# shubhamchandak94/HARC

Hardware: AMD Instinct MI355X
Metric: Mreads/s reorder+encode, 100 bp (higher is better)
Workload: dtype u64 (2-bit packed bases, XOR+popcount)

## Files before the change

harc_amd/csrc/stage1.hip:

```cpp
#include "devutil.h"
#include <stdlib.h>
#include <type_traits>

struct S1Args {
    int L, maxmatch, thresh, maxsearch, Lp;
    int ds[2], de[2], kbits[2];
    uint32_t N, K;
    const uint64_t *reads;
    HashSlot *slots[2];
    uint64_t cap[2];
    const uint32_t *ids[2];
    int firstmax;
    const uint32_t *bloom[2]; uint32_t bloom_lines; int bloom_nwin[2]; uint32_t bloom_mmask;
    const uint2 *largetab;
    uint64_t *mirror;
    unsigned long long *claimed;
    uint32_t *bid;
    ChainHdr *hdr;
    uint4 *cnt;
    uint2 *steps;
    uint8_t *need;
    uint32_t *seedbuf;
    uint32_t *needrank;
    uint32_t *rmeta;
// ... 318 lines not shown
    const bool have = i < nbins;
    auto slot_of = [&](uint32_t k) -> uint64_t { return q[k] - (uint64_t)n + (uint64_t)k; };
    const uint32_t b0 = blockIdx.x * blockDim.x, b1 = b0 + blockDim.x < nbins ? b0 + blockDim.x : nbins;
    bool tiled = false; uint64_t lo = 0, hi = 0;
    if (pass == 0 && fill && b0 < nbins) {
        lo = b0 ? slot_of(b0 - 1) + 1 : 0;
        const uint64_t last = slot_of(b1 - 1);
        if (lo < cap) {
            hi = (last >= cap || b1 == nbins || slot_of(b1) >= cap) ? cap : last + 1;
            tiled = hi - lo <= TP_SPAN;
        }
    }
    if (tiled) {
        const uint4 z = make_uint4(0u, 0u, 0u, 0u);
        for (uint32_t j = threadIdx.x; j < (uint32_t)(hi - lo); j += blockDim.x) tile[j] = z;
        __syncthreads();
    }
    uint64_t sl = have ? slot_of(i) : 0;
    bool mine = have;
    if (mine && pass == 0 && sl >= cap && blockIdx.x + 64 < gridDim.x) { atomicAdd(nbins_p + 1, 1u); mine = false; }
    if (mine && (pass == 1) != (sl >= cap)) mine = false;
    if (mine) {
        const uint32_t st = binstart[i];
        const uint64_t key = skeys[st];
        uint32_t ovf = 0;
        if (pass == 0 && (sl & 3) == 0 && (uint64_t)i + 4 < (uint64_t)nbins) {
            const uint64_t s3 = slot_of(i + 3);
            if (s3 == sl + 3 && (bucket_slot(skeys[binstart[i + 4]], cap) >> 2) <= (sl >> 2)) ovf = SLOT_OVF;
        }
        if (pass == 0 && fill && !tiled) {
            const uint4 z = make_uint4(0u, 0u, 0u, 0u);
            for (uint64_t x = i ? slot_of(i - 1) + 1 : 0; x < sl; x++) *reinterpret_cast<uint4 *>(&slots[x]) = z;
            if (i + 1 == nbins || slot_of(i + 1) >= cap)
                for (uint64_t x = sl + 1; x < cap; x++) *reinterpret_cast<uint4 *>(&slots[x]) = z;
        }
        const uint32_t en = (i + 1 < nbins) ? binstart[i + 1] : n;
        const uint32_t cnt = en - st;
        if (cnt > SLOT_CNT_MASK) atomicAdd(nbins_p + 1, 1u);
        else {
            const unsigned long long meta = cnt == 1 ? ((unsigned long long)sids[st] | ((unsigned long long)(1u | SLOT_EMB) << 32))
                                                     : ((unsigned long long)st | ((unsigned long long)((cnt & SLOT_CNT_MASK) | ((bigthresh && cnt > bigthresh) ? SLOT_BIG : 0u)) << 32));
            if (pass == 1) {
                for (uint64_t bb = bucket_slot(key, cap) >> 2; bb < (cap >> 2); bb++) atomicOr(&slots[4 * bb].count, SLOT_OVF);
                sl = 0;
                for (;;) {
                    unsigned long long *mp = reinterpret_cast<unsigned long long *>(&slots[sl]) + 1;
                    if (atomicCAS(mp, 0ULL, meta) == 0ULL) break;
                    if ((sl & 3) == 3) atomicOr(&slots[sl - 3].count, SLOT_OVF);
                    if (++sl == cap) sl = 0;
                }
                slots[sl].key = key;
            } else {
                uint4 w; w.x = (uint32_t)key; w.y = (uint32_t)(key >> 32); w.z = (uint32_t)meta; w.w = (uint32_t)(meta >> 32) | ovf;
                if (tiled) tile[sl - lo] = w; else *reinterpret_cast<uint4 *>(&slots[sl]) = w;
            }
            if (large_list && cnt > HARC_LARGEBIN) {
                const unsigned int at = atomicAdd(large_n, 1u);
                if (at < large_max) large_list[at] = ((unsigned long long)sl << 1) | large_tag;
            }
        }
    }
    if (tiled) {
        __syncthreads();
        for (uint32_t j = threadIdx.x; j < (uint32_t)(hi - lo); j += blockDim.x) *reinterpret_cast<uint4 *>(&slots[lo + j]) = tile[j];
    }
}

__global__ __launch_bounds__(256) void k_s1_bloom_tile(const uint64_t *pk, uint32_t n, uint64_t nwords, uint32_t *bloom)
{
    __shared__ uint32_t tile[BL_TILE_WORDS];
    __shared__ uint32_t bounds[2];
    const uint32_t part = blockIdx.x;
    for (uint32_t j = threadIdx.x; j < BL_TILE_WORDS; j += 256) tile[j] = 0u;
    if (threadIdx.x < 2) {
        const uint64_t want = (uint64_t)part + threadIdx.x, pmask = ((uint64_t)1 << BL_PART_BITS) - 1;
        uint32_t lo = 0, hi = n;
        while (lo < hi) { const uint32_t mid = lo + (hi - lo) / 2; if ((pk[mid] & pmask) < want) lo = mid + 1; else hi = mid; }
        bounds[threadIdx.x] = lo;
    }
    __syncthreads();
    for (uint32_t i = bounds[0] + threadIdx.x; i < bounds[1]; i += 256) {
        const uint32_t v = (uint32_t)(pk[i] >> BL_PART_BITS);
        atomicOr(&tile[v >> 10], (1u << ((v >> 5) & 31u)) | (1u << (v & 31u)));
    }
    __syncthreads();
    const uint64_t base = (uint64_t)part * BL_TILE_WORDS;
    for (uint32_t j = threadIdx.x; j < BL_TILE_WORDS; j += 256) if (base + j < nwords) bloom[base + j] = tile[j];
}
int harc_bitmap_from_items(harc_amd_ctx *c, const uint64_t *items, uint64_t *tmp, size_t n, uint64_t nwords, uint32_t *bitmap)
{
    const uint64_t ntiles64 = (nwords + BL_TILE_WORDS - 1) / BL_TILE_WORDS;
    if (ntiles64 + 1 >= (1ull << BL_PART_BITS) || n > 0xFFFFFFFFull) { harc_set_error("bitmap of %llu words / %zu items: too large for the tiled build", (unsigned long long)nwords, n); return HARC_AMD_EINVAL; }
    const uint32_t ntiles = (uint32_t)ntiles64;
    if (ntiles == 0) return HARC_AMD_OK;
    unsigned tb = 1; while (((uint64_t)1 << tb) <= ntiles) tb++;
    RC_TRY(prim_sort_keys_u64(c, items, tmp, n, tb));
    hipLaunchKernelGGL(k_s1_bloom_tile, dim3(ntiles), dim3(256), 0, c->stream, (const uint64_t *)tmp, (uint32_t)n, nwords, bitmap);
    HIP_TRY(hipGetLastError());
    return HARC_AMD_OK;
}
__global__ void k_s1_bloom_diff(const uint32_t *a, const uint32_t *b, uint64_t nwords, unsigned long long *ndiff)
{
    const uint64_t i = harc_gid();
    const bool d = i < nwords && a[i] != b[i];
    const unsigned long long m = __ballot(d);
    if ((threadIdx.x & 63) == 0 && m) atomicAdd(ndiff, (unsigned long long)__popcll(m));
}
__global__ void k_s1_bloom_set(const uint64_t *keys, uint32_t n, uint32_t *bloom, uint32_t nlines, int nwin, uint32_t mmask)
{
    const uint32_t i = harc_gid32();
    if (i >= n) return;
    uint32_t w, m;
    bloom_pos(keys[i], key_scramble(keys[i]), nlines, nwin, mmask, &w, &m);
    if ((bloom[w] & m) != m) atomicOr(&bloom[w], m);
}

__global__ void k_init_chains(S1Args s)
{
    const uint32_t c = harc_gid32();
    if (c >= s.K) return;
    ChainHdr h; memset(&h, 0, sizeof h);
    const uint32_t step = s.N / s.K;
    const bool act = s.N > 0 && (c == 0 || step > 0);
    if (act) {
        const uint32_t seed = c * step;
        atomicOr(&s.claimed[seed >> 6], 1ULL << (seed & 63));
        h.cur = seed; h.prev = seed; h.flags = CH_ACTIVE | CH_PREVUNM; h.mode = 2;
    }
    s.hdr[c] = h;
    s.cst2[c] = make_uint2(act ? 1u : 0u, 0u);
    s.need[c] = 0;
    s.pg_cur[c] = c * PG_CHUNK;
    for (uint32_t k = 0; k < PG_CHUNK; k++) s.pg_hdr[(size_t)c * PG_CHUNK + k] = make_uint2(c, k);
    if (c == 0) *s.pg_count = s.K * PG_CHUNK;
}

template <int W, bool INLDS> struct ConsState {
    static constexpr int CT = (W + 1) / 2;
    static constexpr int LP = 64 * CT;
    uint4 qr[INLDS ? 1 : CT];
    uint4 *ql;
    int v[CT];
    int base;
    __device__ __forceinline__ uint4 getq(int t) const { if constexpr (INLDS) return ql[64 * t]; else return qr[t]; }
    __device__ __forceinline__ void setq(int t, const uint4 &q) { if constexpr (INLDS) ql[64 * t] = q; else qr[t] = q; }
};
__device__ __forceinline__ int argmax4(const uint4 &q)
{
    uint32_t mx = 0; int ind = 0;
    if (q.x > mx) { mx = q.x; ind = 0; }
    if (q.y > mx) { mx = q.y; ind = 1; }
    if (q.z > mx) { mx = q.z; ind = 2; }
    if (q.w > mx) { mx = q.w; ind = 3; }
    return ind;
}
template <int W> __device__ __forceinline__ int oriented_base(const uint64_t (&rw)[W], int L, int rev, int i)
{
    const int sc = rev ? (L - 1 - i) : i;
    const int pc = (int)((sel0<W>(rw, sc >> 5) >> (2 * (sc & 31))) & 3);
    const int b = ((pc & 1) << 1) | (pc >> 1);
    return rev ? 3 - b : b;
}
template <int W, bool I> __device__ __forceinline__ void cons_reset(ConsState<W, I> &st, const uint64_t (&rw)[W], int L, int lane)
{
    st.base = 0;
#pragma unroll
    for (int t = 0; t < ConsState<W, I>::CT; t++) {
        const int i = lane + 64 * t;
        int b = 0; uint4 q = make_uint4(0, 0, 0, 0);
        if (i < L) { b = oriented_base<W>(rw, L, 0, i); q.x = (b == 0); q.y = (b == 1); q.z = (b == 2); q.w = (b == 3); }
        st.setq(t, q); st.v[t] = b;
    }
}
template <int W, bool I> __device__ __forceinline__ void cons_update(ConsState<W, I> &st, const uint64_t (&rw)[W], int L, int rev, int shift, int lane)
{
    constexpr int LP = ConsState<W, I>::LP;
    int nb = st.base + shift; if (nb >= LP) nb -= LP;
#pragma unroll
    for (int t = 0; t < ConsState<W, I>::CT; t++) {
        const int p = lane + 64 * t;
        int oldl = p - st.base; if (oldl < 0) oldl += LP;
        int newl = p - nb; if (newl < 0) newl += LP;
        uint4 q = st.getq(t); int v = 0;
        if (newl < L) {
            const int b = oriented_base<W>(rw, L, rev, newl);
            if (oldl < L && oldl >= shift) { q.x += (b == 0); q.y += (b == 1); q.z += (b == 2); q.w += (b == 3); v = argmax4(q); }
            else { q.x = (b == 0); q.y = (b == 1); q.z = (b == 2); q.w = (b == 3); v = b; }
        } else q = make_uint4(0, 0, 0, 0);
        st.setq(t, q); st.v[t] = v;
    }
    st.base = nb;
}
template <int W, bool I> __device__ __forceinline__ void cons_load(ConsState<W, I> &st, const uint4 *src, int L, int lane, uint32_t fmt)
{
    st.base = 0;
#pragma unroll
    for (int t = 0; t < ConsState<W, I>::CT; t++) {
        const int i = lane + 64 * t;
        uint4 q = make_uint4(0, 0, 0, 0); int v = 0;
        if (i < L) {
            if (fmt == 2u) q = src[i];
            else if (fmt == 1u) { const uint2 p = reinterpret_cast<const uint2 *>(src)[i]; q = make_uint4(p.x & 0xFFFFu, p.x >> 16, p.y & 0xFFFFu, p.y >> 16); }
            else { const uint32_t p = reinterpret_cast<const uint32_t *>(src)[i]; q = make_uint4(p & 0xFFu, (p >> 8) & 0xFFu, (p >> 16) & 0xFFu, p >> 24); }
            v = argmax4(q);
        }
        st.setq(t, q); st.v[t] = v;
    }
}
template <int W, bool I> __device__ __forceinline__ uint32_t cons_store(const ConsState<W, I> &st, uint4 *dst, int L, int lane)
{
    constexpr int LP = ConsState<W, I>::LP;
    uint32_t mx = 0;
#pragma unroll
    for (int t = 0; t < ConsState<W, I>::CT; t++) {
        int l = lane + 64 * t - st.base; if (l < 0) l += LP;
        if (l < L) { const uint4 q = st.getq(t); const uint32_t a = q.x > q.y ? q.x : q.y, b = q.z > q.w ? q.z : q.w; const uint32_t m = a > b ? a : b; mx = m > mx ? m : mx; }
    }
    const uint32_t fmt = __ballot(mx > 0xFFFFu) != 0 ? 2u : (__ballot(mx > 0xFFu) != 0 ? 1u : 0u);
#pragma unroll
    for (int t = 0; t < ConsState<W, I>::CT; t++) {
        int l = lane + 64 * t - st.base; if (l < 0) l += LP;
        if (l < L) {
            const uint4 q = st.getq(t);
            if (fmt == 2u) dst[l] = q;
            else if (fmt == 1u) reinterpret_cast<uint2 *>(dst)[l] = make_uint2(q.x | (q.y << 16), q.z | (q.w << 16));
            else reinterpret_cast<uint32_t *>(dst)[l] = q.x | (q.y << 8) | (q.z << 16) | (q.w << 24);
        }
    }
    return fmt;
}
template <int W, bool I> __device__ __forceinline__ void cons_pack(const ConsState<W, I> &st, int L, int lane, uint64_t (&ref)[W])
{
    constexpr int CT = ConsState<W, I>::CT, LP = ConsState<W, I>::LP, RW = 2 * CT;
    uint64_t ring[RW];
#pragma unroll
    for (int t = 0; t < CT; t++) {
        int l = lane + 64 * t - st.base; if (l < 0) l += LP;
        const bool valid = l < L;
        const int v = st.v[t];
        const unsigned long long b0 = __ballot(valid && (v >> 1)), b1 = __ballot(valid && (v & 1));
        ring[2 * t] = spread32(b0) | (spread32(b1) << 1);
        ring[2 * t + 1] = spread32(b0 >> 32) | (spread32(b1 >> 32) << 1);
    }
    const int sb = 2 * st.base, ws = sb >> 6, bs = sb & 63;
#pragma unroll
    for (int w = 0; w < W; w++) {
        int i0 = w + ws; if (i0 >= RW) i0 -= RW;
        int i1 = i0 + 1; if (i1 >= RW) i1 -= RW;
        const uint64_t lo = sel0<RW>(ring, i0), hi = sel0<RW>(ring, i1);
        ref[w] = (bs ? ((lo >> bs) | (hi << (64 - bs))) : lo) & lowmask_word(2 * L, w);
    }
}

#ifndef HARC_STEPS_WAVES
#define HARC_STEPS_WAVES 5
#endif
#ifndef HARC_COOP_WAVES
#define HARC_COOP_WAVES 4
#endif
#ifndef HARC_STEPS_WAVES_Q
#define HARC_STEPS_WAVES_Q 3
#endif
template <int W> struct StepsLds {
    static constexpr int NW = 2 * W;
    static constexpr int ROW = 3 * NW + 1;
    static constexpr int MROW = (NW + 3) & ~3;
};
#ifndef HARC_SEQ_SCAN
#define HARC_SEQ_SCAN 1
#endif
#ifndef HARC_SCAN_CH
#define HARC_SCAN_CH 1
#endif
#define HARC_WGCMD_BYTES 3584
#define HARC_SK_E 4
#ifndef HARC_SCAN_SKETCH
#define HARC_SCAN_SKETCH 1
#endif
#define HARC_OWN_SLOTS 128
#ifndef HARC_SEQ_OWNT
#define HARC_SEQ_OWNT 1
#endif
__device__ __forceinline__ void own_insert(uint32_t *tab, uint32_t id)
{
    uint32_t h = (id * 0x9E3779B1u) >> 25;
    while (tab[h] != HARC_NONE) h = (h + 1u) & (HARC_OWN_SLOTS - 1u);
    tab[h] = id;
}
__device__ __forceinline__ bool own_has(const uint32_t *tab, uint32_t id)
{
    uint32_t h = (id * 0x9E3779B1u) >> 25;
    for (;;) {
        const uint32_t v = tab[h];
        if (v == id) return true;
        if (v == HARC_NONE) return false;
        h = (h + 1u) & (HARC_OWN_SLOTS - 1u);
    }
}
static inline size_t steps_lds_bytes_coop(int W, int maxmatch, int nprobe)
{
    const int NW = 2 * W, ROW = 3 * NW + 1, MROW = (NW + 3) & ~3;
    return ((size_t)2 * maxmatch * MROW + (size_t)((2 * ROW + 3) & ~3) + (size_t)MROW + (size_t)8 * NW + (size_t)32 + (size_t)2 * nprobe + 8) * 4 + HARC_WGCMD_BYTES + 16;
}
static inline size_t steps_lds_bytes(int W, int maxmatch, int nprobe, bool seq = false)
{
    const int NW = 2 * W, ROW = 3 * NW + 1, MROW = (NW + 3) & ~3;
    return (size_t)4 * (64 * ((W + 1) / 2)) * 16 + ((size_t)2 * maxmatch * MROW + (size_t)4 * 2 * ROW + (size_t)4 * MROW + (size_t)4 * 8 * NW + (size_t)4 * 32 + (size_t)(seq ? 4 * HARC_OWN_SLOTS : 0) + (size_t)2 * nprobe + 8) * 4 + 32;
}
template <int W> __device__ __forceinline__ int ham_window(const uint32_t *row, int bitoff, const uint32_t *mrow, const uint32_t (&rd)[2 * W])
{
    constexpr int NW = 2 * W;
    const int i0 = bitoff >> 5, sh = bitoff & 31;
    uint32_t d[NW + 1];
#pragma unroll
    for (int k = 0; k <= NW; k++) d[k] = row[i0 + k];
    int hd = 0;
#pragma unroll
    for (int k = 0; k < NW; k++) hd += __popc((__builtin_amdgcn_alignbit(d[k + 1], d[k], sh) ^ rd[k]) & mrow[k]);
    return hd;
}
template <int W> __device__ __forceinline__ void load_read32(const uint64_t *reads, uint32_t rid, uint32_t (&rd)[2 * W])
{
    if (W % 2 == 0) {
        const uint4 *p = reinterpret_cast<const uint4 *>(reads + (size_t)rid * W);
#pragma unroll
        for (int q = 0; q < W / 2; q++) { const uint4 v = p[q]; rd[4 * q] = v.x; rd[4 * q + 1] = v.y; rd[4 * q + 2] = v.z; rd[4 * q + 3] = v.w; }
    } else {
        const uint2 *p = reinterpret_cast<const uint2 *>(reads + (size_t)rid * W);
#pragma unroll
        for (int q = 0; q < W; q++) { const uint2 v = p[q]; rd[2 * q] = v.x; rd[2 * q + 1] = v.y; }
    }
}
template <int W, bool I> __device__ __forceinline__ void cons_update_lds(ConsState<W, I> &st, const uint32_t *rdl, int L, int rev, int shift, int lane)
{
    constexpr int LP = ConsState<W, I>::LP;
    int nb = st.base + shift; if (nb >= LP) nb -= LP;
#pragma unroll
    for (int t = 0; t < ConsState<W, I>::CT; t++) {
        const int p = lane + 64 * t;
        int oldl = p - st.base; if (oldl < 0) oldl += LP;
        int newl = p - nb; if (newl < 0) newl += LP;
        uint4 q = st.getq(t); int v = 0;
        if (newl < L) {
            const int sc = rev ? (L - 1 - newl) : newl;
            const int pc = (int)((rdl[sc >> 4] >> (2 * (sc & 15))) & 3u);
            int b = ((pc & 1) << 1) | (pc >> 1);
            if (rev) b = 3 - b;
            if (oldl < L && oldl >= shift) { q.x += (b == 0); q.y += (b == 1); q.z += (b == 2); q.w += (b == 3); v = argmax4(q); }
            else { q.x = (b == 0); q.y = (b == 1); q.z = (b == 2); q.w = (b == 3); v = b; }
        } else q = make_uint4(0, 0, 0, 0);
        st.setq(t, q); st.v[t] = v;
    }
    st.base = nb;
}
template <int W, bool I> __device__ __forceinline__ void cons_reset_lds(ConsState<W, I> &st, const uint32_t *rdl, int L, int lane)
{
    st.base = 0;
#pragma unroll
    for (int t = 0; t < ConsState<W, I>::CT; t++) {
        const int i = lane + 64 * t;
        int b = 0; uint4 q = make_uint4(0, 0, 0, 0);
        if (i < L) {
            const int pc = (int)((rdl[i >> 4] >> (2 * (i & 15))) & 3u);
            b = ((pc & 1) << 1) | (pc >> 1);
            q.x = (b == 0); q.y = (b == 1); q.z = (b == 2); q.w = (b == 3);
        }
        st.setq(t, q); st.v[t] = b;
    }
}

template <int W, bool I> __device__ __forceinline__ void cons_rows(const ConsState<W, I> &st, int L, int lane, uint8_t *tmp, uint32_t *rowF, uint32_t *rowR)
{
    constexpr int CT = ConsState<W, I>::CT, LP = ConsState<W, I>::LP, NW = 2 * W;
#pragma unroll
    for (int t = 0; t < CT; t++) {
        int l = lane + 64 * t - st.base; if (l < 0) l += LP;
        if (l < L) {
            const int v = st.v[t];
            const int pc = ((v & 1) << 1) | (v >> 1);
            tmp[l] = (uint8_t)pc;
            tmp[16 * NW + (L - 1 - l)] = (uint8_t)(3 - pc);
        }
    }
    __builtin_amdgcn_fence(__ATOMIC_RELEASE, "wavefront");
    __builtin_amdgcn_wave_barrier();
    if (lane < 2 * NW) {
        const uint4 x = *reinterpret_cast<const uint4 *>(tmp + 16 * lane);
        auto pk = [](uint32_t b) -> uint32_t { b = (b | (b >> 6)) & 0x000F000Fu; return (b | (b >> 12)) & 0xFFu; };
        const uint32_t d = pk(x.x) | (pk(x.y) << 8) | (pk(x.z) << 16) | (pk(x.w) << 24);
        (lane < NW ? rowF + NW + lane : rowR + lane)[0] = d;
    }
    __builtin_amdgcn_fence(__ATOMIC_RELEASE, "wavefront");
    __builtin_amdgcn_wave_barrier();
}

template <int W> __device__ __forceinline__ void rows_from_read(const uint32_t *rdl, int L, int rev, int lane, uint32_t *rowF, uint32_t *rowR)
{
    constexpr int NW = 2 * W;
    int ln = lane; asm volatile("" : "+v"(ln));
    if (ln < 2 * NW) {
        const bool copy = ln < NW;
        const int k = copy ? ln : ln - NW;
        const int P = 2 * (L - 16 * k - 16), i0 = P >> 5;
        const int ia = i0 < 0 ? 0 : (i0 > NW - 1 ? NW - 1 : i0), ib = i0 + 1 < 0 ? 0 : (i0 + 1 > NW - 1 ? NW - 1 : i0 + 1);
        const uint32_t ra = rdl[copy ? k : ia], rb = rdl[ib];
        const uint32_t lo = (i0 >= 0 && i0 < NW) ? ra : 0u, hi = (i0 + 1 >= 0 && i0 + 1 < NW) ? rb : 0u;
        uint32_t w = __brev(__builtin_amdgcn_alignbit(hi, lo, P & 31));
        w = ((w & 0xAAAAAAAAu) >> 1) | ((w & 0x55555555u) << 1);
        const int vb = 2 * L - 32 * k;
        const uint32_t d = copy ? ra : (~w & (vb >= 32 ? 0xFFFFFFFFu : (vb <= 0 ? 0u : ((1u << vb) - 1u))));
        (copy != (rev != 0) ? rowF : rowR)[NW + k] = d;
    }
    __builtin_amdgcn_fence(__ATOMIC_RELEASE, "wavefront");
    __builtin_amdgcn_wave_barrier();
}
template <int W, bool I> __device__ __forceinline__ void cons_flush(ConsState<W, I> &st, const uint16_t *ps, int pend, int ptot, const uint32_t *rowF, int L, int lane)
{
    constexpr int LP = ConsState<W, I>::LP, CT = ConsState<W, I>::CT, NW = 2 * W;
    int nb = 0;
    if (ptot < L) { nb = st.base + ptot; if (nb >= LP) nb -= LP; }
    int ln = lane; asm volatile("" : "+v"(ln));
    int newl[CT], cnt[CT];
#pragma unroll
    for (int t = 0; t < CT; t++) { newl[t] = ln + 64 * t - nb; if (newl[t] < 0) newl[t] += LP; cnt[t] = 0; }
    for (int k = pend - 1; k >= 0; k--) {
        const int d = __builtin_amdgcn_readfirstlane(ptot - (int)ps[k]);
        if (d >= L) break;
#pragma unroll
        for (int t = 0; t < CT; t++) cnt[t] += (d < L - newl[t]) ? 1 : 0;
    }
#pragma unroll
    for (int t = 0; t < CT; t++) {
        uint4 q = make_uint4(0, 0, 0, 0); int v = 0;
        if (newl[t] < L) {
            const int pc = (int)((rowF[NW + (newl[t] >> 4)] >> (2 * (newl[t] & 15))) & 3u);
            v = ((pc & 1) << 1) | (pc >> 1);
            if (newl[t] + ptot < L) q = st.getq(t);
            const uint32_t c = (uint32_t)cnt[t];
            q.x += v == 0 ? c : 0u; q.y += v == 1 ? c : 0u; q.z += v == 2 ? c : 0u; q.w += v == 3 ? c : 0u;
        }
        st.setq(t, q); st.v[t] = v;
    }
    st.base = nb;
}

struct WgCmd {
    int op;
    int l, t, fast;
    uint32_t ids0, m0, cnt;
    uint32_t rot;
    unsigned long long grp;
    uint32_t found;
    uint32_t nc;
    unsigned long long hit[2][HARC_SCAN_CH][4];
    unsigned long long um[2][HARC_SCAN_CH][4];
    uint8_t mj[64], mdir[64];
    uint32_t own[64];
    unsigned long long um4[2][HARC_SK_E][4];
    uint32_t best[2][4];
    uint16_t queue[4][64 * HARC_SK_E];
};
struct WgResult { int besthit, fj, fdir; uint32_t iters, tests, nc;
#ifdef HARC_SKETCH_STATS
    uint32_t rej1, rej2, acc;
#endif
};
static_assert(sizeof(WgCmd) <= HARC_WGCMD_BYTES, "HARC_WGCMD_BYTES too small");
template <int W, int NWV> __device__ __forceinline__ WgResult wg_scan(WgCmd *cmd, int role, int lane, const uint32_t *const *ids, const uint64_t *mirror,
                                                            const uint32_t *rowF, const uint32_t *s_mask, uint32_t *rdl, int maxsearch, int maxmatch, int thresh)
{
    constexpr int NW = StepsLds<W>::NW, ROW = StepsLds<W>::ROW, MROW = StepsLds<W>::MROW, CH = HARC_SCAN_CH;
    WgResult r; r.besthit = 64; r.fj = 0; r.fdir = 0; r.iters = 0; r.tests = 0; r.nc = 0;
#ifdef HARC_SKETCH_STATS
    r.rej1 = r.rej2 = r.acc = 0;
#endif
    const uint32_t *oids = ids[cmd->l];
    const uint32_t ids0 = cmd->ids0, m0 = cmd->m0;
    const int t = cmd->t; const bool fast = cmd->fast != 0;
    unsigned long long grp = cmd->grp;
    int seen = 0, par = 0;
    const uint32_t rot = cmd->rot;
    uint32_t pos = cmd->cnt - rot, lo = 0; bool second = rot == 0;
    uint32_t mrd[CH][NW], rid[CH];
    for (;;) {
        if (pos == lo) { if (second) break; second = true; pos = cmd->cnt; lo = cmd->cnt - rot; }
        if (!(seen < maxsearch && grp)) break;
        bool valid[CH], own[CH], un[CH], cand[CH]; unsigned long long um[CH];
        r.iters++;
#pragma unroll
        for (int c = 0; c < CH; c++) {
            const uint32_t off = 64u * NWV * (uint32_t)c + 64u * (uint32_t)role + (uint32_t)lane;
            valid[c] = off < pos - lo; rid[c] = 0; own[c] = false;
            if (valid[c]) { const uint32_t at = pos - 1 - off; rid[c] = oids[ids0 + at]; load_read32<W>(mirror, m0 + at, mrd[c]); }
        }
        bool ownknown = !fast;
#pragma unroll
        for (int c = 0; c < CH; c++) {
            if (!fast && valid[c]) for (int k = 0; k < t; k++) own[c] |= (cmd->own[k] == rid[c]);
            un[c] = valid[c] && !own[c]; cand[c] = un[c];
            um[c] = __ballot(un[c]);
        }
        int total = 0;
        unsigned long long gm = grp; r.tests += (uint32_t)__popcll(grp);
        bool first = true;
        while (gm) {
            const int g = __ffsll((long long)gm) - 1;
            gm &= gm - 1;
            const int g_j = cmd->mj[g], g_dir = cmd->mdir[g];
            const uint32_t *const omrow = s_mask + (size_t)(g_dir * maxmatch + g_j) * MROW;
            const int obit = g_dir * ROW * 32 + 32 * NW + (g_dir ? -2 * g_j : 2 * g_j);
            bool ok[CH]; bool anyok = false;
#pragma unroll
            for (int c = 0; c < CH; c++) {
                ok[c] = false;
                if (cand[c]) { r.nc++; ok[c] = ham_window<W>(rowF, obit, omrow, mrd[c]) <= thresh; }
#ifdef HARC_SKETCH_STATS
                if (cand[c]) {
                    const int i0 = obit >> 5, sh = obit & 31, k0 = g_dir ? NW - 4 : 0;
                    const int p1 = __popc((__builtin_amdgcn_alignbit(rowF[i0 + k0 + 1], rowF[i0 + k0], sh) ^ mrd[c][k0]) & omrow[k0]);
                    const int p2 = p1 + __popc((__builtin_amdgcn_alignbit(rowF[i0 + k0 + 2], rowF[i0 + k0 + 1], sh) ^ mrd[c][k0 + 1]) & omrow[k0 + 1]);
                    r.rej1 += p1 > thresh; r.rej2 += p2 > thresh; r.acc += ok[c];
                }
#endif
                anyok |= ok[c];
            }
            if (anyok && !ownknown) {
#pragma unroll
                for (int c = 0; c < CH; c++) if (ok[c]) for (int k = 0; k < t; k++) own[c] |= (cmd->own[k] == rid[c]);
                ownknown = true;
            }
#pragma unroll
            for (int c = 0; c < CH; c++) {
                ok[c] = ok[c] && !own[c];
                const unsigned long long pm = __ballot(ok[c]);
                if (lane == 0) { cmd->hit[par][c][role] = pm; if (first && !fast) cmd->um[par][c][role] = um[c]; }
            }
            __syncthreads();
            if (first && !fast) {
                int before[CH];
#pragma unroll
                for (int c = 0; c < CH; c++) {
                    before[c] = total;
                    for (int w = 0; w < NWV; w++) { const int x = __popcll(cmd->um[par][c][w]); if (w < role) before[c] += x; total += x; }
                }
                if (seen + total > maxsearch) {
                    par ^= 1;
#pragma unroll
                    for (int c = 0; c < CH; c++) {
                        cand[c] = un[c] && (seen + before[c] + __popcll(um[c] & ((1ULL << lane) - 1ULL)) < maxsearch);
                        ok[c] = ok[c] && cand[c];
                        const unsigned long long pm = __ballot(ok[c]);
                        if (lane == 0) cmd->hit[par][c][role] = pm;
                    }
                    __syncthreads();
                }
            }
            int winc = -1, winw = 0; unsigned long long winm = 0;
#pragma unroll
            for (int c = CH - 1; c >= 0; c--)
                for (int w = NWV - 1; w >= 0; w--) { const unsigned long long h = cmd->hit[par][c][w]; if (h) { winc = c; winw = w; winm = h; } }
            first = false;
            par ^= 1;
            if (winc >= 0) {
                const int wl = __ffsll((long long)winm) - 1;
                if (role == winw && lane == wl) {
#pragma unroll
                    for (int c = 0; c < CH; c++) if (c == winc) {
#pragma unroll
                        for (int k = 0; k < NW; k++) rdl[k] = mrd[c][k];
                        cmd->found = rid[c];
                    }
                }
                r.fj = g_j; r.fdir = g_dir; r.besthit = g;
                grp &= (1ULL << g) - 1ULL;
                break;
            }
        }
        if (!fast) seen += total;
        pos -= pos - lo > 64u * NWV * CH ? 64u * NWV * CH : pos - lo;
    }
    __syncthreads();
    return r;
}

template <int W, int NWV> __device__ __forceinline__ WgResult wg_scan_sk(WgCmd *cmd, int role, int lane, const uint32_t *const *ids, const uint64_t *mirror,
                                                               const uint32_t *rowF, const uint32_t *s_mask, uint32_t *rdl, int maxsearch, int maxmatch, int thresh)
{
    constexpr int NW = StepsLds<W>::NW, ROW = StepsLds<W>::ROW, MROW = StepsLds<W>::MROW, E = HARC_SK_E;
    constexpr int K0R = NW >= 4 ? NW - 4 : 0;
    WgResult r; r.besthit = 64; r.fj = 0; r.fdir = 0; r.iters = 0; r.tests = 0; r.nc = 0;
#ifdef HARC_SKETCH_STATS
    r.rej1 = r.rej2 = r.acc = 0;
#endif
    const uint32_t *oids = ids[cmd->l];
    const uint32_t ids0 = cmd->ids0, m0 = cmd->m0;
    const int t = cmd->t; const bool fast = cmd->fast != 0;
    unsigned long long grp = cmd->grp;
    uint32_t omin = 0xFFFFFFFFu, omax = 0u;
    for (int k = 0; k < t; k++) { const uint32_t x = cmd->own[k]; omin = x < omin ? x : omin; omax = x > omax ? x : omax; }
    auto is_own = [&](uint32_t rid) -> bool { bool o = false; if (rid >= omin && rid <= omax) for (int k = 0; k < t; k++) o |= (cmd->own[k] == rid); return o; };
    uint16_t *const queue = cmd->queue[role];
    int seen = 0, par = 0;
    const uint32_t rot = cmd->rot;
    uint32_t pos = cmd->cnt - rot, lo = 0; bool second = rot == 0;
    for (;;) {
        if (pos == lo) { if (second) break; second = true; pos = cmd->cnt; lo = cmd->cnt - rot; }
        if (!(seen < maxsearch && grp)) break;
        r.iters++;
        unsigned long long um[E];
        uint2 sk[E];
        const unsigned long long gfirst = grp & (0ULL - grp);
        const int dir0 = cmd->mdir[__ffsll((long long)gfirst) - 1];
#pragma unroll
        for (int e = 0; e < E; e++) {
            const uint32_t off = 64u * (uint32_t)(e * NWV + role) + (uint32_t)lane;
            const bool valid = off < pos - lo;
            bool un = valid; sk[e] = make_uint2(0u, 0u);
            if (valid) {
                const uint32_t at = pos - 1 - off;
                const uint32_t *row = reinterpret_cast<const uint32_t *>(mirror + (size_t)(m0 + at) * W);
                sk[e] = *reinterpret_cast<const uint2 *>(row + (dir0 ? K0R : 0));
                if (!fast && t > 0) un = !is_own(oids[ids0 + at]);
            }
            um[e] = __ballot(un);
        }
        unsigned long long cm[E];
        int total = 0;
#pragma unroll
        for (int e = 0; e < E; e++) cm[e] = um[e];
        if (!fast) {
            if (NWV > 1) {
                if (lane == 0) {
#pragma unroll
                    for (int e = 0; e < E; e++) cmd->um4[par][e][role] = um[e];
                }
                __syncthreads();
            }
            int before[E];
#pragma unroll
            for (int e = 0; e < E; e++) {
                before[e] = total;
                for (int w = 0; w < NWV; w++) { const int x = NWV > 1 ? __popcll(cmd->um4[par][e][w]) : __popcll(um[e]); if (w < role) before[e] += x; total += x; }
            }
            if (NWV > 1) par ^= 1;
            if (seen + total > maxsearch) {
#pragma unroll
                for (int e = 0; e < E; e++) {
                    const int rank = seen + before[e] + __popcll(um[e] & ((1ULL << lane) - 1ULL));
                    cm[e] = __ballot(((um[e] >> lane) & 1ULL) && rank < maxsearch);
                }
            }
        }
        unsigned long long gm = grp; r.tests += (uint32_t)__popcll(grp);
        while (gm) {
            const int g = __ffsll((long long)gm) - 1;
            gm &= gm - 1;
            const int g_j = cmd->mj[g], g_dir = cmd->mdir[g];
            const uint32_t *const omrow = s_mask + (size_t)(g_dir * maxmatch + g_j) * MROW;
            const int obit = g_dir * ROW * 32 + 32 * NW + (g_dir ? -2 * g_j : 2 * g_j);
            unsigned long long sm[E]; int nsurv = 0;
            {
                const int i0 = obit >> 5, sh = obit & 31, k0 = g_dir ? K0R : 0;
                const bool same = g_dir == dir0;
                const uint32_t cA = __builtin_amdgcn_alignbit(rowF[i0 + k0 + 1], rowF[i0 + k0], sh), cB = __builtin_amdgcn_alignbit(rowF[i0 + k0 + 2], rowF[i0 + k0 + 1], sh);
                const uint32_t mA = omrow[k0], mB = omrow[k0 + 1];
#pragma unroll
                for (int e = 0; e < E; e++) {
                    const bool c = (cm[e] >> lane) & 1ULL;
                    const int lb = __popc((cA ^ sk[e].x) & mA) + __popc((cB ^ sk[e].y) & mB);
                    if (c) r.nc++;
                    sm[e] = __ballot(c && (!same || lb <= thresh));
                    if ((sm[e] >> lane) & 1ULL) queue[nsurv + __popcll(sm[e] & ((1ULL << lane) - 1ULL))] = (uint16_t)(64u * (uint32_t)(e * NWV + role) + (uint32_t)lane);
                    nsurv += __popcll(sm[e]);
                }
            }
            __builtin_amdgcn_fence(__ATOMIC_RELEASE, "wavefront");
            __builtin_amdgcn_wave_barrier();
            uint32_t mybest = 0xFFFFFFFFu, myrid = HARC_NONE; uint32_t full[NW];
            for (int b = 0; b < nsurv; b += 64) {
                const int i = b + lane;
                bool ok = false; uint32_t o = 0, rid = 0;
                if (i < nsurv) {
                    o = queue[i];
                    const uint32_t at = pos - 1 - o;
                    load_read32<W>(mirror, m0 + at, full);
                    ok = ham_window<W>(rowF, obit, omrow, full) <= thresh;
                    if (ok) { rid = oids[ids0 + at]; if (fast && t > 0) ok = !is_own(rid); }
#ifdef HARC_SKETCH_STATS
                    r.acc += ok;
#endif
                }
                const unsigned long long pm = __ballot(ok);
                if (pm) {
                    const int wl = __ffsll((long long)pm) - 1;
                    mybest = (uint32_t)__builtin_amdgcn_readlane((int)o, wl);
                    if (lane == wl) myrid = rid; else myrid = HARC_NONE;
                    break;
                }
            }
            uint32_t wbest = mybest; int wrole = role;
            if (NWV > 1) {
                if (lane == 0) cmd->best[par][role] = mybest;
                __syncthreads();
                wbest = 0xFFFFFFFFu; wrole = 0;
                for (int w = 0; w < NWV; w++) { const uint32_t x = cmd->best[par][w]; if (x < wbest) { wbest = x; wrole = w; } }
                par ^= 1;
            }
            if (wbest != 0xFFFFFFFFu) {
                if (role == wrole && myrid != HARC_NONE) {
#pragma unroll
                    for (int k = 0; k < NW; k++) rdl[k] = full[k];
                    cmd->found = myrid;
                }
                r.fj = g_j; r.fdir = g_dir; r.besthit = g;
                grp &= (1ULL << g) - 1ULL;
                break;
            }
        }
        if (!fast) seen += total;
        pos -= pos - lo > 64u * NWV * E ? 64u * NWV * E : pos - lo;
    }
    __syncthreads();
    return r;
}

template <int W> __global__ void k_steps_tables(S1Args s, uint32_t *out)
{
    constexpr int NW = StepsLds<W>::NW, ROW = StepsLds<W>::ROW, MROW = StepsLds<W>::MROW;
    const int L = s.L, nm = 2 * s.maxmatch * MROW;
    for (int i = blockIdx.x * blockDim.x + threadIdx.x; i < nm; i += gridDim.x * blockDim.x) {
        const int k = i % MROW, r = i / MROW, dir = r / s.maxmatch, j = r % s.maxmatch;
        const int lo = dir ? 2 * j : 0, hi = dir ? 2 * L : 2 * (L - j);
        const int a = lo - 32 * k, b = hi - 32 * k;
        const uint32_t mh = b >= 32 ? 0xFFFFFFFFu : (b <= 0 ? 0u : ((1u << b) - 1u)), ml = a >= 32 ? 0xFFFFFFFFu : (a <= 0 ? 0u : ((1u << a) - 1u));
        out[i] = k < NW ? (mh & ~ml) : 0u;
    }
    uint2 *const pinfo = reinterpret_cast<uint2 *>(out + nm);
    for (int i = blockIdx.x * blockDim.x + threadIdx.x; i < s.nprobe; i += gridDim.x * blockDim.x) {
        const uint32_t e = s.probe_tab[i];
        const int j = (int)(e & 0xFF), dir = (int)((e >> 8) & 1), l = (int)((e >> 9) & 1);
        const int koff = dir * ROW * 32 + 32 * NW + (dir ? 2 * (s.ds[l] - j) : 2 * (s.ds[l] + j));
        const int hoff = dir * ROW * 32 + 32 * NW + (dir ? -2 * j : 2 * j);
        pinfo[i] = make_uint2((uint32_t)koff | ((uint32_t)dir << 13) | ((uint32_t)l << 14) | ((uint32_t)j << 16),
                              (uint32_t)hoff | ((uint32_t)((dir * s.maxmatch + j) * MROW) << 16));
    }
}

template <int W> __global__ __launch_bounds__(256) void k_succ(S1Args s, uint2 *succ, uint32_t n)
{
    constexpr int NW = StepsLds<W>::NW, ROW = StepsLds<W>::ROW, MROW = StepsLds<W>::MROW;
    extern __shared__ __attribute__((aligned(16))) uint32_t lds[];
    const int nm = 2 * s.maxmatch * MROW;
    uint32_t *const s_mask = lds;
    uint2 *const s_pinfo = reinterpret_cast<uint2 *>(s_mask + nm);
    uint32_t *const s_rows = reinterpret_cast<uint32_t *>(s_pinfo + s.nprobe);
    uint32_t *const s_rdl = s_rows + 4 * 2 * ROW;
    uint2 *const s_out = reinterpret_cast<uint2 *>(s_rdl + 4 * MROW);
    const int lane = threadIdx.x & 63, wv = threadIdx.x >> 6;
    for (int i = threadIdx.x; i < nm; i += 256) s_mask[i] = s.lds_tab[i];
    { const uint2 *const pt = reinterpret_cast<const uint2 *>(s.lds_tab + nm); for (int i = threadIdx.x; i < s.nprobe; i += 256) s_pinfo[i] = pt[i]; }
    for (int i = threadIdx.x; i < 4 * 2 * ROW; i += 256) s_rows[i] = 0u;
    __syncthreads();
    const uint64_t g = harc_bid() * 4 + wv;
    if (g >= 2ull * n) return;
    const uint32_t r = (uint32_t)(g >> 1); const int o = (int)(g & 1);
    const int L = s.L;
    uint32_t *const rowF = s_rows + (size_t)wv * 2 * ROW, *const rowR = rowF + ROW, *const rdl = s_rdl + (size_t)wv * MROW;
    uint2 *const out = s_out + (size_t)wv * HARC_SUCC_N;
    if (lane < NW) rdl[lane] = reinterpret_cast<const uint32_t *>(s.reads)[(size_t)r * NW + lane];
    if (lane < HARC_SUCC_N) out[lane] = make_uint2(HARC_NONE, 0u);
    __builtin_amdgcn_fence(__ATOMIC_RELEASE, "wavefront");
    __builtin_amdgcn_wave_barrier();
    rows_from_read<W>(rdl, L, o, lane, rowF, rowR);
    const uint64_t kmask0 = s.kbits[0] >= 64 ? ~(uint64_t)0 : (((uint64_t)1 << s.kbits[0]) - 1), kmask1 = s.kbits[1] >= 64 ? ~(uint64_t)0 : (((uint64_t)1 << s.kbits[1]) - 1);
    const uint64_t cap = s.cap[0];
    uint32_t total = 0; bool open = false;
    for (int base = 0; base < s.nprobe && total < HARC_SUCC_N && !open; base += 64) {
        const int p = base + lane;
        int state = 0, j = 0, dir = 0, l = 0; uint32_t sst = 0, cw = 0; uint2 pi = make_uint2(0, 0);
        if (p < s.nprobe && cap) {
            pi = s_pinfo[p];
            j = (int)(pi.x >> 16); dir = (int)((pi.x >> 13) & 1); l = (int)((pi.x >> 14) & 1);
            uint64_t key;
            {
                const int i0 = (int)((pi.x & 0x1FFF) >> 5), shb = (int)(pi.x & 31);
                const uint32_t d0 = rowF[i0], d1 = rowF[i0 + 1], d2 = rowF[i0 + 2];
                key = ((uint64_t)__builtin_amdgcn_alignbit(d1, d0, shb) | ((uint64_t)__builtin_amdgcn_alignbit(d2, d1, shb) << 32)) & (l ? kmask1 : kmask0);
            }
            const HashSlot *const tab = l ? s.slots[1] : s.slots[0];
            const uint64_t hk = key_scramble(key);
            uint64_t sl = bucket_slot(hk, cap);
            if (s.bloom_lines) {
                uint32_t bw, bm;
                bloom_pos(key, hk, s.bloom_lines, s.bloom_nwin[0], s.bloom_mmask, &bw, &bm);
                if (((l ? s.bloom[1] : s.bloom[0])[bw] & bm) != bm) state = 1;
            }
            while (state == 0) {
                uint32_t w0 = 0;
#pragma unroll
                for (int q = 0; q < 4; q++) {
                    const uint4 raw = *reinterpret_cast<const uint4 *>(&tab[sl + q]);
                    if (q == 0) w0 = raw.w;
                    if (state == 0) {
                        if (raw.w == 0) state = 1;
                        else if (raw.x == (uint32_t)hk && raw.y == (uint32_t)(hk >> 32)) { state = 2; sst = raw.z; cw = raw.w; }
                    }
                }
                if (state == 0 && !(w0 & SLOT_OVF)) state = 1;
                sl += 4; if (sl >= cap) sl = 0;
            }
        }
        const bool big = state == 2 && (cw & SLOT_BIG) != 0;
        const unsigned long long mb = __ballot(big);
        const int firstbig = mb ? __ffsll((long long)mb) - 1 : 64;
        const bool scan = state == 2 && !big && lane < firstbig;
        const uint32_t cntb = cw & SLOT_CNT_MASK; const bool emb = (cw & SLOT_EMB) != 0;
        const uint32_t *const ids = l ? s.ids[1] : s.ids[0];
        const uint32_t *const mrow = s_mask + (pi.y >> 16);
        const int bitoff = (int)(pi.y & 0xFFFF);
        uint32_t cnt = 0;
        if (scan) for (uint32_t i = cntb; i > 0; i--) {
            const uint32_t rid = emb ? sst : ids[sst + i - 1];
            if (rid == r) continue;
            uint32_t mrd[NW];
            load_read32<W>(s.reads, rid, mrd);
            if (ham_window<W>(rowF, bitoff, mrow, mrd) <= s.thresh) cnt++;
        }
        uint32_t incl = cnt;
        for (int d = 1; d < 64; d <<= 1) { const uint32_t y = (uint32_t)__shfl_up((int)incl, d, 64); if (lane >= d) incl += y; }
        const uint32_t off = total + incl - cnt;
        if (scan && cnt && off < HARC_SUCC_N) {
            uint32_t k = 0;
            for (uint32_t i = cntb; i > 0; i--) {
                const uint32_t rid = emb ? sst : ids[sst + i - 1];
                if (rid == r) continue;
                uint32_t mrd[NW];
                load_read32<W>(s.reads, rid, mrd);
                const int hd = ham_window<W>(rowF, bitoff, mrow, mrd);
                if (hd <= s.thresh) { if (off + k < HARC_SUCC_N) out[off + k] = make_uint2(rid, (uint32_t)j | ((uint32_t)dir << 8) | ((uint32_t)hd << 9) | ((uint32_t)p << 16)); k++; }
            }
        }
        total += (uint32_t)__shfl((int)incl, 63, 64);
        if (firstbig < 64) open = true;
    }
    if (total >= HARC_SUCC_N) open = true;
    __builtin_amdgcn_fence(__ATOMIC_RELEASE, "wavefront");
    __builtin_amdgcn_wave_barrier();
    if (lane < HARC_SUCC_N) { uint2 e = out[lane]; if (open) e.y |= HARC_SUCC_OPEN; succ[g * HARC_SUCC_N + lane] = e; }
}
static inline size_t succ_lds_bytes(int W, int maxmatch, int nprobe)
{
    const int NW = 2 * W, ROW = 3 * NW + 1, MROW = (NW + 3) & ~3;
    return ((size_t)2 * maxmatch * MROW + (size_t)2 * nprobe + (size_t)4 * 2 * ROW + (size_t)4 * MROW + (size_t)4 * HARC_SUCC_N * 2) * 4 + 16;
}

template <int W, bool QUAD, bool COOP, int NWV = 4, bool SEQ = false, bool SPEC = false> __global__ __launch_bounds__(256, COOP ? HARC_COOP_WAVES : (QUAD ? HARC_STEPS_WAVES_Q : (W <= 4 ? HARC_STEPS_WAVES : HARC_STEPS_WAVES - 1) + (SEQ ? HARC_SEQ_EXTRA_WAVES : 2))) void k_steps(S1Args s)
{
    constexpr int NW = StepsLds<W>::NW, ROW = StepsLds<W>::ROW, MROW = StepsLds<W>::MROW;
    extern __shared__ __attribute__((aligned(16))) uint32_t lds[];
    constexpr int NSL = COOP ? 1 : 4;
    uint32_t *const s_mask = lds + (COOP ? (size_t)0 : (size_t)4 * ConsState<W, !QUAD>::LP * 4);
    uint32_t *const s_rows = s_mask + (size_t)2 * s.maxmatch * MROW;
    uint32_t *const s_rdl = s_rows + ((NSL * 2 * ROW + 3) & ~3);
    uint32_t *const s_tmp = s_rdl + NSL * MROW;
    uint32_t *const s_pend = s_tmp + NSL * 8 * NW;
    uint32_t *const s_own = s_pend + NSL * 32;
    constexpr bool OWNT = (SEQ && HARC_SEQ_OWNT) || (QUAD && !COOP);
    uint2 *const s_pinfo = reinterpret_cast<uint2 *>(s_own + (OWNT ? 4 * HARC_OWN_SLOTS : 0));
    WgCmd *const cmd = reinterpret_cast<WgCmd *>(reinterpret_cast<char *>(s_pinfo + s.nprobe) + 8 - ((size_t)(s_pinfo + s.nprobe) & 7));
    const int lane = threadIdx.x & 63, role = threadIdx.x >> 6, wv = COOP ? 0 : role;
    const int L = s.L;
    if (s.own_mod > 1 && ((COOP ? (blockIdx.x >> 2) : blockIdx.x) % s.own_mod) != s.own_rem) return;
    if (COOP) {
        if (blockIdx.x >= s.K) return;
        const uint32_t fl = s.hdr[blockIdx.x].flags;
        if (!(fl & CH_ACTIVE) || !(fl & CH_COOP)) return;
    }
    {
        const int nm = 2 * s.maxmatch * MROW;
        for (int i = threadIdx.x; i < nm; i += 64 * NWV) s_mask[i] = s.lds_tab[i];
        const uint2 *const pt = reinterpret_cast<const uint2 *>(s.lds_tab + nm);
        for (int i = threadIdx.x; i < s.nprobe; i += 64 * NWV) s_pinfo[i] = pt[i];
        for (int i = threadIdx.x; i < NSL * 2 * ROW; i += 64 * NWV) s_rows[i] = 0u;
        for (int i = threadIdx.x; i < NSL * 8 * NW; i += 64 * NWV) s_tmp[i] = 0u;
        if constexpr (OWNT) for (int i = threadIdx.x; i < 4 * HARC_OWN_SLOTS; i += 64 * NWV) s_own[i] = HARC_NONE;
        __syncthreads();
    }
    if (COOP && role != 0) {
        const uint32_t *const idp[2] = { s.ids[0], s.ids[1] };
        uint32_t hnc = 0;
        for (;;) {
            __syncthreads();
            if (cmd->op == 0) break;
            const WgResult r = (HARC_SCAN_SKETCH && NWV == 1) ? wg_scan_sk<W, NWV>(cmd, role, lane, idp, s.mirror, s_rows, s_mask, s_rdl, s.maxsearch, s.maxmatch, s.thresh)
                                                : wg_scan<W, NWV>(cmd, role, lane, idp, s.mirror, s_rows, s_mask, s_rdl, s.maxsearch, s.maxmatch, s.thresh);
            hnc += r.nc;
#ifdef HARC_SKETCH_STATS
            if (s.dbg) { const uint32_t a1 = wave_sum_u32(r.rej1), a2 = wave_sum_u32(r.rej2), a3 = wave_sum_u32(r.acc), a0 = wave_sum_u32(r.nc); if (lane == 0) { atomicAdd(&s.dbg[44], (unsigned long long)a0); atomicAdd(&s.dbg[45], (unsigned long long)a1); atomicAdd(&s.dbg[46], (unsigned long long)a2); atomicAdd(&s.dbg[47], (unsigned long long)a3); } }
#endif
        }
        hnc = wave_sum_u32(hnc);
        if (lane == 0 && hnc) { atomicAdd(&s.cstat_coop[blockIdx.x].y, hnc); atomicAdd(&s.cstat_coop[blockIdx.x].w, hnc); }
        return;
    }
    const long long dbg_t0 = (COOP && s.dbg) ? wall_clock64() : 0;
#ifdef HARC_COOP_TRACE
    long long dbg_tl = dbg_t0; unsigned long long dbg_ph[6] = { 0, 0, 0, 0, 0, 0 }, dbg_kt[4] = { 0, 0, 0, 0 }, dbg_kn[4] = { 0, 0, 0, 0 };
#define PH(k) do { if (COOP && s.dbg) { const long long tn_ = wall_clock64(); dbg_ph[k] += (unsigned long long)(tn_ - dbg_tl); dbg_tl = tn_; } } while (0)
#else
#define PH(k) do { } while (0)
#endif
    uint32_t ownreg = HARC_NONE;
    const uint32_t c = COOP ? blockIdx.x : (uint32_t)__builtin_amdgcn_readfirstlane((int)(blockIdx.x * 4 + wv));
    if (c >= s.K) return;
    ChainHdr h;
    {
        const uint4 *hp = reinterpret_cast<const uint4 *>(&s.hdr[c]);
        const uint4 h0 = hp[0], h1 = hp[1];
        h.cur = (uint32_t)__builtin_amdgcn_readfirstlane((int)h0.x); h.prev = (uint32_t)__builtin_amdgcn_readfirstlane((int)h0.y);
        h.flags = (uint32_t)__builtin_amdgcn_readfirstlane((int)h0.z); h.mode = (uint32_t)__builtin_amdgcn_readfirstlane((int)h0.w);
        h.n_main = (uint32_t)__builtin_amdgcn_readfirstlane((int)h1.x); h.n_sing = (uint32_t)__builtin_amdgcn_readfirstlane((int)h1.y);
        h.nsteps = (uint32_t)__builtin_amdgcn_readfirstlane((int)h1.z); h.pad0 = (uint32_t)__builtin_amdgcn_readfirstlane((int)h1.w);
    }
    uint4 cst = s.cstat[c];
    cst.x = (uint32_t)__builtin_amdgcn_readfirstlane((int)cst.x); cst.y = (uint32_t)__builtin_amdgcn_readfirstlane((int)cst.y);
    cst.z = (uint32_t)__builtin_amdgcn_readfirstlane((int)cst.z); cst.w = (uint32_t)__builtin_amdgcn_readfirstlane((int)cst.w);
    if (!(h.flags & CH_ACTIVE)) return;
    if (!COOP && s.bo && (s.bo[c] & 0xFFu)) return;
    if (COOP && !(h.flags & CH_COOP)) return;
    if (!COOP && s.need[c]) {
        const uint32_t r = s.needrank[c], R = s.rmeta[0], assigned = s.rmeta[1], got = s.rmeta[2];
        if (h.flags & CH_PREVUNM) {
            if (lane == 0) s.slog[h.prev] = make_uint2(c, h.n_sing);
            h.n_sing++;
        }
        if (r < assigned) {
            const uint32_t id = s.seedbuf[r];
            h.cur = id; h.prev = id; h.flags = ((h.flags | CH_PREVUNM) & ~CH_NEEDSEED) & 0xFFFFu; h.mode = 2;
            const uint32_t first = r * (uint32_t)s.nsugg_per_seed;
            const uint32_t ng = first >= got ? 0u : (got - first < (uint32_t)s.nsugg_per_seed ? got - first : (uint32_t)s.nsugg_per_seed);
            if ((uint32_t)lane < ng) s.sugg[(size_t)c * s.nsugg_stride + lane] = s.seedbuf[R + first + lane];
            h.nsteps = ng << 24;
            if (lane == 0) { uint2 q = s.cst2[c]; q.x++; s.cst2[c] = q; s.need[c] = 0; }
        } else {
            h.flags &= ~(CH_ACTIVE | CH_PREVUNM | CH_NEEDSEED);
            if (lane == 0) { atomicAdd(&s.stats[ST_ACTIVE], ~0ULL); s.need[c] = 0; s.hdr[c] = h; }
            return;
        }
    }
    constexpr int LP = ConsState<W, !QUAD>::LP;
    const uint32_t par = (h.flags & CH_PARITY) ? 1u : 0u;
    uint4 *B0 = s.cnt + ((size_t)par * s.K + c) * LP;
    uint4 *B1 = s.cnt + ((size_t)(par ^ 1u) * s.K + c) * LP;
    ConsState<W, !QUAD> st;
    st.ql = reinterpret_cast<uint4 *>(lds) + (size_t)wv * ConsState<W, !QUAD>::LP + lane;
    const int T0 = COOP ? (int)(h.nsteps & 0xFF) : 0;
    if (COOP) {
        cons_load(st, T0 > 0 ? B1 : B0, L, lane, (h.pad0 >> (24 + 2 * (T0 > 0 ? (par ^ 1u) : par))) & 3u);
        if (lane < T0) ownreg = s.steps[(size_t)c * 64 + lane].x;
    } else if (h.mode == 2) {
        uint64_t rw[W];
#pragma unroll
        for (int w = 0; w < W; w++) rw[w] = s.reads[(size_t)h.cur * W + w];
        cons_reset(st, rw, L, lane);
    } else {
        cons_load(st, B0, L, lane, (h.pad0 >> (24 + 2 * par)) & 3u);
        if (h.mode == 1) {
            const int nrep = (int)((h.nsteps >> 8) & 0xFF);
            uint2 sp = make_uint2(0, 0);
            uint64_t mrw[W];
#pragma unroll
            for (int w = 0; w < W; w++) mrw[w] = 0;
            if (lane < nrep) {
                sp = s.steps[(size_t)c * 64 + lane];
#pragma unroll
                for (int w = 0; w < W; w++) mrw[w] = s.reads[(size_t)sp.x * W + w];
            }
            for (int t = 0; t < nrep; t++) {
                uint64_t rw[W];
#pragma unroll
                for (int w = 0; w < W; w++) rw[w] = shfl_u64(mrw[w], t);
                const uint32_t y = __shfl(sp.y, t, 64);
                if ((y >> 16) & 1) cons_reset(st, rw, L, lane);
                else cons_update(st, rw, L, (int)((y >> 8) & 1), (int)(y & 0xFF), lane);
            }
        }
    }
    uint32_t widebits = (h.pad0 >> 24) & 15u;
    if (!COOP && h.mode != 0) { const uint32_t w0 = cons_store(st, B0, L, lane); widebits = (widebits & ~(3u << (2 * par))) | (w0 << (2 * par)); }

    uint32_t *const rowF = s_rows + (size_t)wv * 2 * ROW, *const rowR = rowF + ROW, *const rdl = s_rdl + (size_t)wv * MROW;
    uint8_t *const coltmp = reinterpret_cast<uint8_t *>(s_tmp + (size_t)wv * 8 * NW);
    uint32_t *const ownt = s_own + (size_t)wv * HARC_OWN_SLOTS;
    uint16_t *const pshift = reinterpret_cast<uint16_t *>(s_pend + (size_t)wv * 32);
    const uint64_t kmask0 = (SPEC || s.kbits[0] >= 64) ? ~(uint64_t)0 : (((uint64_t)1 << s.kbits[0]) - 1), kmask1 = (SPEC || s.kbits[1] >= 64) ? ~(uint64_t)0 : (((uint64_t)1 << s.kbits[1]) - 1);
    const uint64_t cap = s.cap[0];
    uint32_t dbg_bins = 0, dbg_iter = 0, dbg_miss = 0, dbg_surv = 0, dbg_batches = 0;
    uint32_t np = 0, nc = 0, nuse = 0, ncu = 0;
    using flag_t = typename std::conditional<SEQ, int, bool>::type;
    int nst = 0; flag_t needseed = false, defer = false;
    int lastp = (int)(h.pad0 & 0xFFFF);
    int spos = (int)((h.nsteps >> 16) & 0xFF); const int nsugg = (int)(h.nsteps >> 24);
    int bigprobes = 0;
    const int resume = (int)(h.flags >> 16);
    flag_t stalled = false; int resume_next = 0;
    flag_t rows_ok = false; int pend = 0, ptot = 0;
    const flag_t lazy = (SEQ || (QUAD && !COOP)) && s.lazy != 0;
    constexpr bool FASTP = QUAD && !COOP;
    uint32_t lastrid = HARC_NONE; int lastdir = 0; bool rows_lazy = false;
    uint2 enext = make_uint2(HARC_NONE, 0u); bool have_next = false;
    const bool ownlate = FASTP && s.succ != nullptr;
    int own_ins = T0;
    auto own_sync = [&](int upto) {
        if (lane >= own_ins && lane < upto) {
            uint32_t hh = (ownreg * 0x9E3779B1u) >> 25;
            while (atomicCAS(&ownt[hh], HARC_NONE, ownreg) != HARC_NONE) hh = (hh + 1u) & (HARC_OWN_SLOTS - 1u);
        }
        own_ins = upto;
        __builtin_amdgcn_fence(__ATOMIC_RELEASE, "wavefront");
        __builtin_amdgcn_wave_barrier();
    };
    uint32_t seedrid = HARC_NONE;
    auto counts_sync = [&]() {
        if (seedrid == HARC_NONE) return;
        if (lane < NW) rdl[lane] = reinterpret_cast<const uint32_t *>(s.reads)[(size_t)seedrid * NW + lane];
        __builtin_amdgcn_fence(__ATOMIC_RELEASE, "wavefront");
        __builtin_amdgcn_wave_barrier();
        cons_reset_lds(st, rdl, L, lane);
        seedrid = HARC_NONE;
        __builtin_amdgcn_fence(__ATOMIC_RELEASE, "wavefront");
        __builtin_amdgcn_wave_barrier();
    };
    if (FASTP && s.succ && h.mode == 2) lastrid = h.cur;
    auto rows_materialise = [&]() {
        if (lane < NW) rdl[lane] = reinterpret_cast<const uint32_t *>(s.reads)[(size_t)lastrid * NW + lane];
        __builtin_amdgcn_fence(__ATOMIC_RELEASE, "wavefront");
        __builtin_amdgcn_wave_barrier();
        rows_from_read<W>(rdl, L, lastdir, lane, rowF, rowR);
        rows_ok = true; rows_lazy = false;
    };
    PH(0);
    for (int t = T0; t < s.S; t++) {
        uint32_t found = HARC_NONE; int fj = 0, fdir = 0, fhd = -1;
        bool viafast = false, nohit = false;
        if constexpr (FASTP) {
            if (s.succ && lastrid != HARC_NONE && !(t == 0 && resume > 0)) {
                uint2 e = make_uint2(HARC_NONE, 0u);
                if (have_next) e = enext;
                else if (lane < HARC_SUCC_N) e = s.succ[((size_t)lastrid * 2 + (size_t)lastdir) * HARC_SUCC_N + lane];
                have_next = false;
                static_assert(HARC_SUCC_N == 8, "lane >> 3 = entry, lane & 7 = entry of its list");
                const uint32_t ck = (uint32_t)__shfl((int)e.x, lane >> 3, 64), cy = (uint32_t)__shfl((int)e.y, lane >> 3, 64);
                uint2 e2 = make_uint2(HARC_NONE, 0u);
                if (ck != HARC_NONE) e2 = s.succ[((size_t)ck * 2 + (size_t)((cy >> 8) & 1u)) * HARC_SUCC_N + (lane & 7)];
                bool ok = false;
                if (e.x != HARC_NONE) ok = !((s.claimed[e.x >> 6] >> (e.x & 63)) & 1ULL);
                unsigned long long m = __ballot(ok);
                while (m) {
                    const uint32_t x = (uint32_t)__builtin_amdgcn_readlane((int)e.x, __ffsll((long long)m) - 1);
                    if (!__ballot(ownreg == x)) break;
                    m &= m - 1ULL;
                }
                if (m) {
                    const int f = __ffsll((long long)m) - 1;
                    enext.x = (uint32_t)__shfl((int)e2.x, 8 * f + (lane & 7), 64); enext.y = (uint32_t)__shfl((int)e2.y, 8 * f + (lane & 7), 64);
                    if (lane >= HARC_SUCC_N) enext = make_uint2(HARC_NONE, 0u);
                    found = (uint32_t)__builtin_amdgcn_readlane((int)e.x, f);
                    const uint32_t meta = (uint32_t)__builtin_amdgcn_readlane((int)e.y, f);
                    fj = (int)(meta & 0xFFu); fdir = (int)((meta >> 8) & 1u); fhd = (int)((meta >> 9) & 0x7Fu);
                    const int pp = (int)((meta >> 16) & 0xFFFu);
                    nuse += (uint32_t)(pp + 1); lastp += 4 * pp - (lastp >> 2);
                    if (lane == 0) { nc++; ncu++; }
                    viafast = true; have_next = fhd == 0;
                } else if (!((uint32_t)__builtin_amdgcn_readlane((int)e.y, 0) & HARC_SUCC_OPEN)) nohit = true;
            }
        }
        if (!viafast && !nohit) {
        if (ownlate && own_ins < t) own_sync(t);
        if (ownlate) counts_sync();
        if (!rows_ok) { if (FASTP && rows_lazy) rows_materialise(); else cons_rows(st, L, lane, coltmp, rowF, rowR); }
        PH(1);
        int base = (t == 0 && resume > 0) ? resume : 0;
        int stepbig = 0;
        for (int bi = 0; base < s.nprobe; bi++) {
            int bend;
            { int w0 = bi == 0 ? ((HARC_W0_MUL * (lastp >> 4) + HARC_W0_ADD + 15) & ~15) : 64; const int wmax = (QUAD || SPEC) ? 64 : (bi <= 1 ? s.firstmax : 64); if (w0 > wmax) w0 = wmax; bend = base + w0; }
            if (bend > s.nprobe) bend = s.nprobe;
            if (bend <= base) bend = s.nprobe;
            const int p = base + lane; dbg_batches++;
            uint32_t mine = HARC_NONE; int j = 0, dir = 0, l = 0, myhd = 0;
            uint32_t pix = 0;
            uint32_t ncb = 0;
            bool big = false; uint32_t b_cnt = 0; uint64_t b_slot = 0;
            uint2 b_lt = make_uint2(0, 0);
            bool cand = false; uint32_t c_sst = 0, c_cw = 0, c_piy = 0; uint64_t c_slot = 0;
            uint32_t mrd[NW];
            if (p < bend && (SPEC || cap)) {
                const uint2 pi = s_pinfo[p];
                pix = pi.x;
                j = (int)(pi.x >> 16); dir = (int)((pi.x >> 13) & 1);
                l = (int)((pi.x >> 14) & 1);
                uint64_t key;
                {
                    const int i0 = (int)((pi.x & 0x1FFF) >> 5), shb = (int)(pi.x & 31);
                    const uint32_t d0 = rowF[i0], d1 = rowF[i0 + 1], d2 = rowF[i0 + 2];
                    key = (uint64_t)__builtin_amdgcn_alignbit(d1, d0, shb) | ((uint64_t)__builtin_amdgcn_alignbit(d2, d1, shb) << 32);
                    if constexpr (!SPEC) key &= (l ? kmask1 : kmask0);
                }
                HashSlot *const tab = l ? s.slots[1] : s.slots[0];
                uint32_t hmid, hlo = key_scramble_lo(key, &hmid);
                uint64_t hk = 0, sl = 0;
                if constexpr (!SEQ) {
                    hk = key_scramble_hi(hlo, hmid);
                    sl = bucket_slot(hk, cap);
                }
                int state = 0, qhit = 0;
                uint32_t sst = 0, cw = 0;
                if (SPEC || s.bloom_lines) {
                    uint32_t bw, bm;
                    if constexpr (SPEC) bloom_pos(key, hlo, s.bloom_lines, 17, 0xFFFFFFFFu, &bw, &bm);
                    else bloom_pos(key, hlo, s.bloom_lines, s.bloom_nwin[0], s.bloom_mmask, &bw, &bm);
                    if (((l ? s.bloom[1] : s.bloom[0])[bw] & bm) != bm) state = 1;
                }
                if (SEQ && state == 0) {
                    asm volatile("" : "+v"(hlo));
                    hk = key_scramble_hi(hlo, hmid);
                    if constexpr (SPEC) sl = (uint64_t)__umulhi((uint32_t)(hk >> 32), (uint32_t)(cap >> 2)) << 2; else sl = bucket_slot(hk, cap);
                }
                if (state == 0) for (;;) {
                    constexpr int NQ = QUAD ? 4 : 2;
                    uint32_t w0 = 0;
#pragma unroll
                    for (int hp = 0; hp < 4 / NQ; hp++) {
                        if (state == 0) {
                            uint4 rawq[NQ];
#pragma unroll
                            for (int q = 0; q < NQ; q++) rawq[q] = *reinterpret_cast<const uint4 *>(&tab[sl + hp * NQ + q]);
                            if constexpr (SEQ) {
#pragma unroll
                                for (int q = 0; q < NQ; q++) asm volatile("" : "+v"(rawq[q].x), "+v"(rawq[q].y), "+v"(rawq[q].z), "+v"(rawq[q].w));
                                if (hp == 0) w0 = rawq[0].w;
#pragma unroll
                                for (int q = 0; q < NQ; q++) {
                                    const bool live = state == 0;
                                    const bool em = rawq[q].w == 0, mt = (rawq[q].x == (uint32_t)hk) & (rawq[q].y == (uint32_t)(hk >> 32)) & !em;
                                    np += live ? 1u : 0u;
                                    qhit = (live & mt) ? hp * NQ + q : qhit; sst = (live & mt) ? rawq[q].z : sst; cw = (live & mt) ? rawq[q].w : cw;
                                    state = live ? (em ? 1 : (mt ? 2 : 0)) : state;
                                }
                            } else {
                                if (hp == 0) w0 = rawq[0].w;
#pragma unroll
                                for (int q = 0; q < NQ; q++) {
                                    if (state == 0) {
                                        np++;
                                        if (rawq[q].w == 0) state = 1;
                                        else if (rawq[q].x == (uint32_t)hk && rawq[q].y == (uint32_t)(hk >> 32)) { state = 2; qhit = hp * NQ + q; sst = rawq[q].z; cw = rawq[q].w; }
                                    }
                                }
                            }
                        }
                    }
                    if (state == 0 && !(w0 & SLOT_OVF)) state = 1;
                    if (state) break;
                    sl += 4; if (sl >= cap) sl = 0;
                }
                if (state == 2 && !(cw & SLOT_DEAD)) {
                    if (cw & SLOT_BIG) { big = true; b_cnt = cw & (SLOT_CNT_MASK | SLOT_OVF | SLOT_BIG); b_slot = sl + qhit; if (COOP) b_lt = s.largetab[sst]; }
                    else if constexpr (SEQ) {
                        cand = true; c_sst = sst; c_cw = cw; c_piy = pi.y; c_slot = sl + qhit;
                        if (cw & SLOT_EMB) {
                            if (__popcll(__ballot(true)) >= s.weedmin && ((reinterpret_cast<const uint32_t *>(s.claimed)[sst >> 5] >> (sst & 31u)) & 1u)) { cand = false; atomicOr(reinterpret_cast<uint32_t *>(&tab[sl + qhit]) + 3, SLOT_DEAD); }
                            else if (OWNT && own_has(ownt, sst)) cand = false;
                        }
                    }
                    else {
                        const uint32_t cntb = cw & SLOT_CNT_MASK;
                        const bool emb = (cw & SLOT_EMB) != 0;
                        const uint32_t *const ids = l ? s.ids[1] : s.ids[0];
                        const uint32_t *const mrow = s_mask + (pi.y >> 16);
                        const int bitoff = (int)(pi.y & 0xFFFF);
                        const bool exactwin = !SPEC && s.maxsearch < (int)HARC_LARGEBIN;
                        uint32_t lead = 0; bool alltop = true; int seen = 0;
                        for (uint32_t i = cntb; i > 0 && seen < s.maxsearch; i--) {
                            const uint32_t rid = emb ? sst : ids[sst + i - 1];
                            const unsigned long long cwd = s.claimed[rid >> 6];
                            load_read32<W>(s.reads, rid, mrd);
                            if ((cwd >> (rid & 63)) & 1ULL) { if (alltop) lead++; continue; }
                            alltop = false;
                            const int hd = ham_window<W>(rowF, bitoff, mrow, mrd);
                            bool own = false;
                            if (exactwin || hd <= s.thresh) {
                                if constexpr (OWNT) own = own_has(ownt, rid);
                                else for (int k = 0; k < t; k++) own |= ((uint32_t)__builtin_amdgcn_readlane((int)ownreg, k) == rid);
                            }
                            if (own) continue;
                            nc++; ncb++; if (exactwin) seen++;
                            if (hd <= s.thresh) { mine = rid; myhd = hd; break; }
                        }
                        if (lead) {
                            uint32_t *cp = reinterpret_cast<uint32_t *>(&tab[sl + qhit]) + 3;
                            if (lead == cntb) atomicOr(cp, SLOT_DEAD); else if (!emb) atomicMin(cp, (cntb - lead) | (cw & SLOT_OVF));
                        }
                    }
                }
            }
            int winlane = 64;
            if constexpr (SEQ) {
            {
                unsigned long long mc = __ballot(cand);
                if (!COOP) { const unsigned long long mb = __ballot(big); if (mb) mc &= (mb & (0ULL - mb)) - 1ULL; }
                const bool exactwin = !SPEC && s.maxsearch < (int)HARC_LARGEBIN;
                uint32_t ntest = 0;
                while (mc) {
                    const int w = __ffsll((long long)mc) - 1;
                    mc &= mc - 1ULL;
                    const uint32_t o_sst = (uint32_t)__builtin_amdgcn_readlane((int)c_sst, w), o_cw = (uint32_t)__builtin_amdgcn_readlane((int)c_cw, w);
                    const uint32_t o_piy = (uint32_t)__builtin_amdgcn_readlane((int)c_piy, w);
                    const uint32_t o_pix = (uint32_t)__builtin_amdgcn_readlane((int)pix, w);
                    const int o_l = (int)((o_pix >> 14) & 1);
                    const uint32_t cntb = o_cw & SLOT_CNT_MASK;
                    const bool emb = (o_cw & SLOT_EMB) != 0;
                    const uint32_t *const ids = o_l ? s.ids[1] : s.ids[0];
                    const int bitoff = (int)(o_piy & 0xFFFF), i0 = bitoff >> 5, sh = bitoff & 31;
                    const uint32_t *const mrow = s_mask + (o_piy >> 16);
                    const uint64_t o_slot = (uint64_t)(uint32_t)__builtin_amdgcn_readlane((int)(uint32_t)c_slot, w) | ((uint64_t)(uint32_t)__builtin_amdgcn_readlane((int)(uint32_t)(c_slot >> 32), w) << 32);
                    uint32_t lead = 0, hit = HARC_NONE, rd = 0; bool alltop = true; int seen = 0, hit_hd = -1;
                    uint32_t idv = 0;
                    if (!emb && (uint32_t)lane < cntb) idv = ids[o_sst + lane];
                    for (uint32_t i = cntb; i > 0 && seen < s.maxsearch; i--) {
                        const uint32_t rid = emb ? o_sst : (uint32_t)__builtin_amdgcn_readlane((int)idv, (int)(i - 1));
                        if (!OWNT && __ballot(ownreg == rid && lane < t)) { alltop = false; continue; }
                        const uint32_t cwv = reinterpret_cast<const uint32_t *>(s.claimed)[rid >> 5];
                        rd = lane < NW ? reinterpret_cast<const uint32_t *>(s.reads)[(size_t)rid * NW + lane] : 0u;
                        const uint32_t cwd = (uint32_t)__builtin_amdgcn_readfirstlane((int)cwv);
                        if ((cwd >> (rid & 31u)) & 1u) { if (alltop) lead++; continue; }
                        alltop = false;
                        if (OWNT && __ballot(ownreg == rid && lane < t)) continue;
                        uint32_t hdp = 0;
                        if (lane < NW) hdp = (uint32_t)__popc((__builtin_amdgcn_alignbit(rowF[i0 + lane + 1], rowF[i0 + lane], sh) ^ rd) & mrow[lane]);
                        hdp += (uint32_t)__builtin_amdgcn_update_dpp(0, (int)hdp, 0x118, 0xF, 0xF, true);
                        hdp += (uint32_t)__builtin_amdgcn_update_dpp(0, (int)hdp, 0x114, 0xF, 0xF, true);
                        hdp += (uint32_t)__builtin_amdgcn_update_dpp(0, (int)hdp, 0x112, 0xF, 0xF, true);
                        hdp += (uint32_t)__builtin_amdgcn_update_dpp(0, (int)hdp, 0x111, 0xF, 0xF, true);
                        const int hd = __builtin_amdgcn_readlane((int)hdp, 15);
                        ntest++; if (exactwin) seen++;
                        if (hd <= s.thresh) { hit = rid; hit_hd = hd; break; }
                    }
                    if (lead && lane == 0) {
                        uint32_t *cp = reinterpret_cast<uint32_t *>(&(o_l ? s.slots[1] : s.slots[0])[o_slot]) + 3;
                        if (lead == cntb) atomicOr(cp, SLOT_DEAD); else if (!emb) atomicMin(cp, (cntb - lead) | (o_cw & SLOT_OVF));
                    }
                    if (hit != HARC_NONE) {
                        winlane = w; found = hit; fj = (int)(o_pix >> 16); fdir = (int)((o_pix >> 13) & 1); fhd = hit_hd;
                        if (lane < NW) rdl[lane] = rd;
                        break;
                    }
                }
                if (lane == 0) { nc += ntest; ncu += ntest; }
            }
            } else {
                const unsigned long long msmall = __ballot(mine != HARC_NONE);
                if (msmall) {
                    winlane = __ffsll((long long)msmall) - 1;
                    found = (uint32_t)__builtin_amdgcn_readlane((int)mine, winlane); fj = __builtin_amdgcn_readlane(j, winlane); fdir = __builtin_amdgcn_readlane(dir, winlane);
                    fhd = __builtin_amdgcn_readlane(myhd, winlane);
                    if (lane == winlane) {
#pragma unroll
                        for (int k = 0; k < NW; k++) rdl[k] = mrd[k];
                    }
                }
            }
            PH(2);
            {
                const unsigned long long bigall = __ballot(big);
                unsigned long long bigm = bigall;
                if (winlane < 64) bigm &= (1ULL << winlane) - 1ULL;
                if (!COOP) { if (bigm) { defer = true; break; } }
                int caplane = 64;
                if (COOP) {
                    const int need = s.stepcap - stepbig;
                    if (need >= 1 && __popcll(bigall) >= need) { unsigned long long m = bigall; for (int k = 1; k < need; k++) m &= m - 1; caplane = __ffsll((long long)m) - 1; }
                    if (caplane < 64 && caplane < winlane) bigm &= (2ULL << caplane) - 1ULL;
                }
                if (COOP) while (bigm) {
                    const int bl = __ffsll((long long)bigm) - 1;
                    const uint32_t o_raw = (uint32_t)__builtin_amdgcn_readlane((int)b_cnt, bl), o_cnt = o_raw & SLOT_CNT_MASK;
                    const int o_l = __builtin_amdgcn_readlane(l, bl);
                    const uint64_t o_slot = shfl_u64(b_slot, bl);
                    unsigned long long grp = __ballot(big && l == o_l && b_slot == o_slot) & bigm;
                    bigm &= ~grp;
                    dbg_bins++;
#ifdef HARC_COOP_TRACE
                    const int dbg_kind = o_cnt <= 64 ? 0 : o_cnt <= 256 ? 1 : o_cnt <= 1024 ? 2 : 3;
                    const long long dbg_s0 = s.dbg ? wall_clock64() : 0;
#endif
                    const uint2 lt = make_uint2((uint32_t)__builtin_amdgcn_readlane((int)b_lt.x, bl), (uint32_t)__builtin_amdgcn_readlane((int)b_lt.y, bl));
                    cmd->mj[lane] = (uint8_t)j; cmd->mdir[lane] = (uint8_t)dir; cmd->own[lane] = ownreg;
                    if (lane == 0) {
                        cmd->op = 1; cmd->l = o_l; cmd->t = t; cmd->fast = o_cnt <= (uint32_t)s.maxsearch ? 1 : 0;
                        cmd->ids0 = lt.x; cmd->m0 = lt.y; cmd->cnt = o_cnt; cmd->grp = grp; cmd->found = HARC_NONE;
                        { const uint32_t m = o_cnt < (uint32_t)s.maxsearch ? o_cnt : (uint32_t)s.maxsearch; cmd->rot = m ? ((c * 0x9E3779B1u) >> 8) % m : 0u; }
                    }
                    __syncthreads();
                    const uint32_t *const idp[2] = { s.ids[0], s.ids[1] };
                    const WgResult wr = (HARC_SCAN_SKETCH && NWV == 1) ? wg_scan_sk<W, NWV>(cmd, 0, lane, idp, s.mirror, rowF, s_mask, rdl, s.maxsearch, s.maxmatch, s.thresh)
                                                         : wg_scan<W, NWV>(cmd, 0, lane, idp, s.mirror, rowF, s_mask, rdl, s.maxsearch, s.maxmatch, s.thresh);
                    dbg_iter += wr.iters; dbg_surv += wr.tests; nc += wr.nc; ncu += wr.nc;
#ifdef HARC_SKETCH_STATS
                    if (s.dbg) { const uint32_t a1 = wave_sum_u32(wr.rej1), a2 = wave_sum_u32(wr.rej2), a3 = wave_sum_u32(wr.acc), a0 = wave_sum_u32(wr.nc); if (lane == 0) { atomicAdd(&s.dbg[44], (unsigned long long)a0); atomicAdd(&s.dbg[45], (unsigned long long)a1); atomicAdd(&s.dbg[46], (unsigned long long)a2); atomicAdd(&s.dbg[47], (unsigned long long)a3); } }
#endif
                    const int besthit = wr.besthit;
                    if (besthit < 64) { found = cmd->found; fj = wr.fj; fdir = wr.fdir; fhd = -1; }
                    if (besthit < 64) { winlane = besthit; bigm &= (1ULL << besthit) - 1ULL; }
#ifdef HARC_COOP_TRACE
                    if (s.dbg) { dbg_kt[dbg_kind] += (unsigned long long)(wall_clock64() - dbg_s0); dbg_kn[dbg_kind]++; }
#endif
                }
                if (COOP && caplane < 64 && caplane < winlane) {
                    stalled = true; resume_next = base + caplane + 1;
                    break;
                }
                if (COOP) { const int nb = __popcll(bigall & (winlane < 64 ? ((2ULL << winlane) - 1ULL) : ~0ULL)); bigprobes += nb; stepbig += nb; }
            }
            PH(3);
            if (lane <= winlane) ncu += ncb;
            if (found != HARC_NONE) {
                nuse += (uint32_t)(base + winlane + 1);
                lastp += 4 * (base + winlane) - (lastp >> 2);
                break;
            }
            base = bend;
        }
        }
        if (defer || stalled) break;
        if (found == HARC_NONE) {
            nuse += (uint32_t)s.nprobe; dbg_miss++;
            if (ownlate && own_ins < t) own_sync(t);
            uint32_t sid = HARC_NONE;
            if (spos < nsugg) {
                const int idx = spos + lane;
                uint32_t id = 0; bool okc = false;
                if (idx < nsugg) {
                    id = __hip_atomic_load(&s.sugg[(size_t)c * s.nsugg_stride + idx], __ATOMIC_RELAXED, __HIP_MEMORY_SCOPE_AGENT);
                    okc = !((s.claimed[id >> 6] >> (id & 63)) & 1ULL);
                    if constexpr (OWNT) okc = okc && !own_has(ownt, id);
                    else for (int k = 0; k < t; k++) okc = okc && ((uint32_t)__builtin_amdgcn_readlane((int)ownreg, k) != id);
                }
                const unsigned long long sm = __ballot(okc);
                if (sm) { const int f = __ffsll((long long)sm) - 1; sid = __shfl(id, f, 64); spos += f + 1; } else spos = nsugg;
            }
            if (sid == HARC_NONE) { needseed = true; break; }
            if (lane == 0) s.steps[(size_t)c * 64 + t] = make_uint2(sid, (1u << 16) | ((uint32_t)spos << 24));
            if (lane == t) ownreg = sid;
            if constexpr (OWNT) { if (!ownlate && lane == 0) own_insert(ownt, sid); __builtin_amdgcn_fence(__ATOMIC_RELEASE, "wavefront"); }
            if (ownlate) { seedrid = sid; lastrid = sid; lastdir = 0; rows_lazy = true; }
            else {
                if (lane < NW) { const uint32_t *rp = reinterpret_cast<const uint32_t *>(s.reads + (size_t)sid * W); rdl[lane] = rp[lane]; }
                __builtin_amdgcn_fence(__ATOMIC_RELEASE, "wavefront");
                __builtin_amdgcn_wave_barrier();
                cons_reset_lds(st, rdl, L, lane);
            }
            rows_ok = false; pend = 0; ptot = 0;
            nst++;
            if (COOP && bigprobes >= s.budget) break;
            continue;
        }
        if (lane == 0) s.steps[(size_t)c * 64 + t] = make_uint2(found, (uint32_t)fj | ((uint32_t)fdir << 8));
        if (lane == t) ownreg = found;
        if constexpr (OWNT) { if (!ownlate && lane == 0) own_insert(ownt, found); }
        __builtin_amdgcn_fence(__ATOMIC_RELEASE, "wavefront");
        __builtin_amdgcn_wave_barrier();
        if (FASTP && viafast && fhd == 0) {
            ptot += fj;
            if (lane == 0) pshift[pend] = (uint16_t)ptot;
            pend++; rows_ok = false; rows_lazy = true; lastrid = found; lastdir = fdir;
        } else {
            if (FASTP && viafast) {
                counts_sync();
                if (pend && !rows_ok) rows_materialise();
                if (lane < NW) rdl[lane] = reinterpret_cast<const uint32_t *>(s.reads)[(size_t)found * NW + lane];
                __builtin_amdgcn_fence(__ATOMIC_RELEASE, "wavefront");
                __builtin_amdgcn_wave_barrier();
            }
            if (lazy && fhd == 0) {
                rows_from_read<W>(rdl, L, fdir, lane, rowF, rowR);
                ptot += fj;
                if (lane == 0) pshift[pend] = (uint16_t)ptot;
                pend++; rows_ok = true;
                if (FASTP && s.succ) { lastrid = found; lastdir = fdir; rows_lazy = false; }
            } else {
                if (pend) { __builtin_amdgcn_fence(__ATOMIC_RELEASE, "wavefront"); __builtin_amdgcn_wave_barrier(); cons_flush(st, pshift, pend, ptot, rowF, L, lane); pend = 0; ptot = 0; }
                cons_update_lds(st, rdl, L, fdir, fj, lane);
                rows_ok = false;
                if (FASTP) { lastrid = HARC_NONE; rows_lazy = false; }
            }
        }
        nst++;
        PH(4);
        if (COOP && bigprobes >= s.budget) break;
    }
    if (lane >= T0 && lane < T0 + nst) atomicMin(&s.bid[ownreg], ((uint32_t)lane << 20) | c);
    if (ownlate) counts_sync();
    if (pend) {
        if (FASTP && rows_lazy) rows_materialise();
        __builtin_amdgcn_fence(__ATOMIC_RELEASE, "wavefront"); __builtin_amdgcn_wave_barrier(); cons_flush(st, pshift, pend, ptot, rowF, L, lane); pend = 0; ptot = 0;
    }
    PH(4);
    if (COOP) { if (lane == 0) cmd->op = 0; __syncthreads(); }
    if (nst > 0) { const uint32_t w1 = cons_store(st, B1, L, lane); widebits = (widebits & ~(3u << (2 * (par ^ 1u)))) | (w1 << (2 * (par ^ 1u))); }
    np = wave_sum_u32(np); nc = wave_sum_u32(nc); ncu = wave_sum_u32(ncu);
    PH(5);
#undef PH
#ifdef HARC_COOP_TRACE
    if (COOP && lane == 0 && s.dbg) {
        for (int k = 0; k < 6; k++) atomicAdd(&s.dbg[16 + k], dbg_ph[k]);
        for (int k = 0; k < 4; k++) { atomicAdd(&s.dbg[36 + k], dbg_kn[k]); atomicAdd(&s.dbg[40 + k], dbg_kt[k]); }
        const unsigned long long dt0 = (unsigned long long)(wall_clock64() - dbg_t0);
        atomicAdd(&s.dbg[24 + (dt0 / 2500 < 11 ? dt0 / 2500 : 11)], 1ULL);
    }
#endif
    if (COOP && lane == 0 && s.dbg) { const unsigned long long dt = (unsigned long long)(wall_clock64() - dbg_t0); atomicAdd(&s.dbg[9], 1ULL); atomicAdd(&s.dbg[10], dt); atomicMax(&s.dbg[11], dt); atomicAdd(&s.dbg[12], (unsigned long long)(nst)); }
    if (!COOP && lane == 0 && s.dbg) { atomicAdd(&s.dbg[13], 1ULL); if (defer) atomicAdd(&s.dbg[15], 1ULL); if (defer && nst == 0) atomicAdd(&s.dbg[14], 1ULL); }
    if (lane == 0 && s.dbg) { atomicAdd(&s.dbg[0], (unsigned long long)dbg_bins); atomicAdd(&s.dbg[1], (unsigned long long)dbg_iter); atomicAdd(&s.dbg[2], (unsigned long long)dbg_miss); atomicAdd(&s.dbg[3], (unsigned long long)dbg_surv); atomicAdd(&s.dbg[4], (unsigned long long)nst); atomicAdd(&s.dbg[5], (unsigned long long)dbg_batches); atomicMax(&s.dbg[6], (unsigned long long)dbg_iter); atomicMax(&s.dbg[7], (unsigned long long)dbg_surv); atomicMax(&s.dbg[8], (unsigned long long)dbg_bins); }
    if (lane == 0) {
        if (COOP) { atomicAdd(&s.cstat_coop[c].x, np); atomicAdd(&s.cstat_coop[c].y, nc); atomicAdd(&s.cstat_coop[c].z, nuse); atomicAdd(&s.cstat_coop[c].w, ncu); s.csteps[c].y += (uint32_t)nst; }
        else { cst.x += np; cst.y += nc; cst.z += nuse; cst.w += ncu; s.cstat[c] = cst; s.csteps[c].x += (uint32_t)nst; }
        h.mode = 0;
        h.nsteps = (h.nsteps & 0xFFFF0000u) | (uint32_t)(T0 + nst);
        h.pad0 = ((uint32_t)lastp & 0xFFFFu) | (((uint32_t)spos & 0xFFu) << 16) | (widebits << 24);
        h.flags = needseed ? (h.flags | CH_NEEDSEED) : (h.flags & ~CH_NEEDSEED);
        h.flags = defer ? (h.flags | CH_COOP) : (h.flags & ~CH_COOP);
        h.flags = (h.flags & 0xFFFFu) | ((COOP ? (stalled ? (uint32_t)resume_next : 0u) : ((defer && nst == 0) ? (uint32_t)resume : 0u)) << 16);
        if (!COOP && defer) atomicAdd(&s.coopcnt[c & (HARC_COOPCNT - 1)], 1ULL);
        s.hdr[c] = h;
    }
}

__device__ __forceinline__ bool chain_owned(uint32_t c, uint32_t mod, uint32_t rem) { return mod <= 1 || ((c >> 2) % mod) == rem; }
__global__ void k_apply_seed(S1Args s)
{
    const uint32_t c = harc_gid32();
    if (c >= s.K || chain_owned(c, s.own_mod, s.own_rem)) return;
    ChainHdr h = s.hdr[c];
    if (!(h.flags & CH_ACTIVE) || !s.need[c]) return;
    const uint32_t r = s.needrank[c], R = s.rmeta[0], assigned = s.rmeta[1], got = s.rmeta[2];
    if (h.flags & CH_PREVUNM) {
        s.slog[h.prev] = make_uint2(c, h.n_sing);
        h.n_sing++;
    }
    if (r < assigned) {
        const uint32_t id = s.seedbuf[r];
        h.cur = id; h.prev = id; h.flags = ((h.flags | CH_PREVUNM) & ~CH_NEEDSEED) & 0xFFFFu; h.mode = 2;
        const uint32_t first = r * (uint32_t)s.nsugg_per_seed;
        const uint32_t ng = first >= got ? 0u : (got - first < (uint32_t)s.nsugg_per_seed ? got - first : (uint32_t)s.nsugg_per_seed);
        for (uint32_t k = 0; k < ng; k++) s.sugg[(size_t)c * s.nsugg_stride + k] = s.seedbuf[R + first + k];
        h.nsteps = ng << 24;
        uint2 q = s.cst2[c]; q.x++; s.cst2[c] = q;
    } else {
        h.flags &= ~(CH_ACTIVE | CH_PREVUNM | CH_NEEDSEED);
        atomicAdd(&s.stats[ST_ACTIVE], ~0ULL);
    }
    s.need[c] = 0;
    s.hdr[c] = h;
}
__global__ void k_pack_chains(S1Args s, uint32_t *buf, uint32_t nper)
{
    const uint32_t recw = 8u + 2u * (uint32_t)s.S;
    const uint64_t gid = harc_gid();
    if (gid >= (uint64_t)nper * recw) return;
    const uint32_t li = (uint32_t)(gid / recw), d = (uint32_t)(gid % recw);
    const uint32_t c = ((li >> 2) * s.own_mod + s.own_rem) * 4u + (li & 3u);
    uint32_t v = 0;
    if (c < s.K) v = d < 8u ? reinterpret_cast<const uint32_t *>(&s.hdr[c])[d] : reinterpret_cast<const uint32_t *>(&s.steps[(size_t)c * 64])[d - 8u];
    buf[gid] = v;
}
__global__ void k_unpack_chains(S1Args s, const uint32_t *buf, uint32_t nper)
{
    const uint32_t recw = 8u + 2u * (uint32_t)s.S, p = blockIdx.y;
    if (p == s.own_rem) return;
    const uint64_t gid = (uint64_t)blockIdx.x * blockDim.x + threadIdx.x;
    if (gid >= (uint64_t)nper * recw) return;
    const uint32_t li = (uint32_t)(gid / recw), d = (uint32_t)(gid % recw);
    const uint32_t c = ((li >> 2) * s.own_mod + p) * 4u + (li & 3u);
    if (c >= s.K) return;
    const uint32_t *rec = buf + ((size_t)p * nper + li) * recw;
    const uint32_t v = rec[d];
    if (d < 8u) reinterpret_cast<uint32_t *>(&s.hdr[c])[d] = v;
    else {
        reinterpret_cast<uint32_t *>(&s.steps[(size_t)c * 64])[d - 8u] = v;
        const uint32_t t = (d - 8u) >> 1;
        if (((d - 8u) & 1u) == 0 && (rec[2] & CH_ACTIVE) && t < (rec[6] & 0xFFu)) atomicMin(&s.bid[v], (t << 20) | c);
    }
}

__device__ __forceinline__ unsigned long long wave_sum_u64(unsigned long long v) { for (int o = 32; o > 0; o >>= 1) v += shfl_u64(v, (__lane_id() + o) & 63); return v; }
__device__ __forceinline__ unsigned long long digest_mix(unsigned long long x) { x ^= x >> 33; x *= 0xff51afd7ed558ccdULL; x ^= x >> 33; x *= 0xc4ceb9fe1a85ec53ULL; return x ^ (x >> 33); }
__global__ void k_replica_digest(S1Args s, unsigned long long nwords, unsigned long long *out)
{
    const unsigned long long gid = (unsigned long long)blockIdx.x * blockDim.x + threadIdx.x, nth = (unsigned long long)gridDim.x * blockDim.x;
    unsigned long long a = 0, b = 0, d = 0;
    for (unsigned long long i = gid; i < nwords; i += nth) { const unsigned long long w = s.claimed[i]; if (w) a += digest_mix(w ^ (i * 0x9E3779B97F4A7C15ULL)); }
    for (unsigned long long i = gid; i < (unsigned long long)s.K * 8; i += nth) b += digest_mix((unsigned long long)reinterpret_cast<const uint32_t *>(s.hdr)[i] ^ (i * 0x9E3779B97F4A7C15ULL));
    for (unsigned long long i = gid; i < s.K; i += nth) if (s.need[i]) d += digest_mix(i + 1);
    a = wave_sum_u64(a); b = wave_sum_u64(b); d = wave_sum_u64(d);
    if ((threadIdx.x & 63) == 0) { if (a) atomicAdd(&out[0], a); if (b) atomicAdd(&out[1], b); if (d) atomicAdd(&out[2], d); }
    if (gid == 0) { out[3] = (unsigned long long)*s.cursor; out[4] = s.rmeta[0]; out[5] = s.rmeta[1]; out[6] = s.rmeta[2]; }
}

template <int G> __device__ __forceinline__ void resolve_body(const S1Args &s, const uint32_t bx)
{
    constexpr int CPW = 64 / G;
    const int lane = threadIdx.x & 63, sub = lane / G, sl = lane % G, g0 = sub * G;
    if (bx == 0 && threadIdx.x == 0) { s.reseed_g[0] = 0u; s.reseed_g[1] = 0u; }
    const uint32_t c = (bx * 4 + (threadIdx.x >> 6)) * CPW + sub;
    ChainHdr h; h.flags = 0; h.nsteps = 0; h.n_main = 0; h.n_sing = 0; h.prev = 0; h.pad0 = 0;
    if (c < s.K) h = s.hdr[c];
    const uint32_t bo0 = (s.bo && c < s.K) ? s.bo[c] : 0u;
    const bool asleep = (bo0 & 0xFFu) != 0;
    if (asleep && sl == 0) s.bo[c] = bo0 - 1u;
    const bool act = c < s.K && (h.flags & CH_ACTIVE) && !asleep;
    const int n = act ? (int)(h.nsteps & 0xFF) : 0;
    uint2 sp = make_uint2(HARC_NONE, 0);
    bool mineb = false;
    if (sl < n) {
        sp = s.steps[(size_t)c * 64 + sl];
        mineb = s.bid[sp.x] == (((uint32_t)sl << 20) | c);
    }
    unsigned long long lost = __ballot(sl < n && !mineb);
    if (G < 64) lost = (lost >> g0) & ((1ULL << (G & 63)) - 1ULL);
    const int v = lost ? (__ffsll((long long)lost) - 1) : n;
    const bool cut = v < n;
    const bool kept = sl < v;
    if (mineb && !kept) s.bid[sp.x] = HARC_NONE;
    const bool seedk = kept && ((sp.y >> 16) & 1);
    const uint32_t pkind = __shfl_up((uint32_t)seedk, 1, 64), prid = __shfl_up(sp.x, 1, 64);
    const bool punm = sl == 0 ? ((h.flags & CH_PREVUNM) != 0) : (pkind != 0);
    const uint32_t pid = sl == 0 ? h.prev : prid;
    const uint32_t nm = kept ? (seedk ? 0u : (punm ? 2u : 1u)) : 0u;
    const uint32_t ns = (kept && seedk && punm) ? 1u : 0u;
    uint32_t tm, ts;
    const uint32_t em = wave_excl_scan_u32(nm, &tm), es = wave_excl_scan_u32(ns, &ts);
    const uint32_t em0 = __shfl(em, g0, 64), es0 = __shfl(es, g0, 64);
    const int lastl = g0 + (v > 0 ? v - 1 : 0);
    const uint32_t gm = __shfl(em + nm, lastl, 64) - em0, gs = __shfl(es + ns, lastl, 64) - es0;
    uint32_t pcur = 0, pnew = 0, qcur = 0, qlast = 0;
    bool wantchunk = false;
    if (act && sl == 0 && v > 0 && gm > 0) {
        pcur = s.pg_cur[c];
        qcur = ((h.n_main ? h.n_main - 1u : 0u) >> 6) / PG_CHUNK;
        qlast = ((h.n_main + gm - 1u) >> 6) / PG_CHUNK;
        wantchunk = qlast != qcur;
    }
    {
        __shared__ uint32_t sh_cnt, sh_base;
        if (__syncthreads_or(wantchunk ? 1 : 0)) {
            if (threadIdx.x == 0) sh_cnt = 0u;
            __syncthreads();
            uint32_t myrank = 0;
            if (wantchunk) myrank = atomicAdd(&sh_cnt, 1u);
            __syncthreads();
            if (threadIdx.x == 0) sh_base = atomicAdd(s.pg_count, sh_cnt * (unsigned int)PG_CHUNK);
            __syncthreads();
            if (wantchunk) {
                pnew = sh_base + myrank * PG_CHUNK;
                for (uint32_t k = 0; k < PG_CHUNK; k++) s.pg_hdr[pnew + k] = make_uint2(c, qlast * PG_CHUNK + k);
                s.pg_cur[c] = pnew;
            }
        }
    }
    pcur = __shfl(pcur, g0, 64); pnew = __shfl(pnew, g0, 64); qcur = __shfl(qcur, g0, 64);
    if (kept) {
        atomicOr(&s.claimed[sp.x >> 6], 1ULL << (sp.x & 63));
        if (seedk) {
            if (punm) s.slog[pid] = make_uint2(c, h.n_sing + (es - es0));
        } else {
            uint32_t seq = h.n_main + (em - em0);
            if (punm) {
                const uint32_t pn = seq >> 6, pg = (pn / PG_CHUNK == qcur ? pcur : pnew) + pn % PG_CHUNK;
                s.pg_rec[(size_t)pg * 64 + (seq & 63u)] = make_uint2(pid, (uint32_t)(s.L & 0xFF));
                seq++;
            }
            const uint32_t pn = seq >> 6, pg = (pn / PG_CHUNK == qcur ? pcur : pnew) + pn % PG_CHUNK;
            s.pg_rec[(size_t)pg * 64 + (seq & 63u)] = make_uint2(sp.x, (sp.y & 0xFF) | (1u << 8) | (((sp.y >> 8) & 1u) << 9));
        }
    }
    const uint32_t lastrid = __shfl(sp.x, lastl, 64), lastseed = __shfl((uint32_t)seedk, lastl, 64);
    unsigned long long seedmask = __ballot(seedk);
    if (G < 64) seedmask = (seedmask >> g0) & ((1ULL << (G & 63)) - 1ULL);
    const int nseed = __popcll(seedmask);
    const int lastseedlane = seedmask ? (63 - __clzll((long long)seedmask)) : 0;
    const uint32_t lastsidx = __shfl(sp.y >> 24, g0 + lastseedlane, 64);
    if (act && sl == 0) {
        if (v > 0) {
            h.n_main += gm; h.n_sing += gs;
            h.cur = lastrid;
            if (lastseed) { h.prev = lastrid; h.flags |= CH_PREVUNM; } else h.flags &= ~CH_PREVUNM;
        }
        uint32_t spos = (h.nsteps >> 16) & 0xFF;
        if (cut) { if (nseed) spos = lastsidx; }
        else spos = (h.pad0 >> 16) & 0xFF;
        const uint32_t keep = (h.nsteps & 0xFF000000u) | (spos << 16);
        if (cut) {
            h.mode = v > 0 ? 1u : 0u; h.nsteps = keep | ((uint32_t)v << 8); h.flags &= ~CH_NEEDSEED; h.flags &= 0xFFFFu;
        } else {
            if (n > 0) { h.flags ^= CH_PARITY; h.mode = 0; }
            h.nsteps = keep;
        }
        s.hdr[c] = h;
        if (nseed || cut) { uint2 q = s.cst2[c]; q.x += (uint32_t)nseed; q.y += cut ? 1u : 0u; s.cst2[c] = q; }
        s.need[c] = (!cut && (h.flags & CH_NEEDSEED)) ? 1 : 0;
        if (s.bo) {
            uint32_t k = (bo0 >> 8) & 0xFFu, zs = 0u;
            if (cut) { if (k < HARC_BO_FREE + HARC_BO_CAP) k++; zs = k > HARC_BO_FREE ? (1u << (k - HARC_BO_FREE)) - 1u : 0u; }
            else if (n > 0) k = 0;
            s.bo[c] = zs | (k << 8);
        }
    }
}
template <int G> __global__ __launch_bounds__(256) void k_resolve(S1Args s) { resolve_body<G>(s, blockIdx.x); }

template <int NT> __device__ __forceinline__ void reseed_body(const S1Args &s)
{
    __shared__ uint32_t sm[20];
    __shared__ long long scursor;
    const int t = threadIdx.x;
    const uint32_t chunk = (((s.K + NT - 1) / NT) + 7) & ~7u;
    const uint32_t c0 = (uint32_t)t * chunk;
    uint32_t mycnt = 0;
    if (c0 < s.K) for (uint32_t c = c0; c < c0 + chunk; c += 8) mycnt += (uint32_t)__popcll(*(const unsigned long long *)(s.need + c));
    uint32_t R; const uint32_t rbase = block_excl_scan_u32<NT>(mycnt, sm, &R);
    if (R == 0) return;
    if (mycnt) {
        uint32_t r = rbase;
        for (uint32_t c = c0; c < c0 + chunk; c += 8) {
            unsigned long long w = *(const unsigned long long *)(s.need + c);
            while (w) { const int b = __ffsll((long long)w) - 1; w &= w - 1; s.needrank[c + (uint32_t)(b >> 3)] = r++; }
        }
    }

    long long cursor = *s.cursor;
    uint32_t assigned = 0;
    while (assigned < R && cursor >= 0) {
        const long long cwd = cursor >> 6, wi = cwd - t;
        unsigned long long bits = 0;
        if (wi >= 0) {
            bits = ~s.claimed[wi];
            if (wi == cwd) { const int top = (int)(cursor & 63); if (top < 63) bits &= (2ULL << top) - 1ULL; }
        }
        uint32_t total; const uint32_t off = block_excl_scan_u32<NT>((uint32_t)__popcll(bits), sm, &total);
        unsigned long long newclaim = 0; uint32_t k = 0;
        while (bits && assigned + off + k < R) {
            const int b = 63 - __clzll((long long)bits);
            bits &= ~(1ULL << b);
            const uint32_t id = (uint32_t)(wi * 64 + b), r = assigned + off + k;
            k++; newclaim |= 1ULL << b;
            s.seedbuf[r] = id;
            if (r == R - 1) scursor = (long long)id - 1;
        }
        if (newclaim) s.claimed[wi] |= newclaim;
        __syncthreads();
        if (assigned + total >= R) { assigned = R; cursor = scursor; }
        else { assigned += total; cursor = (cwd - (NT - 1)) * 64 - 1; }
        __syncthreads();
    }
    const uint32_t want = assigned * (uint32_t)s.nsugg_per_seed;
    uint32_t got = 0;
    const long long look = cursor;
    __threadfence();
    __syncthreads();
    if (look < 0) got = want;
    for (int ch = 0; ch < HARC_LOOK_CHUNKS * (1024 / NT) && got < want; ch++) {
        const long long cwd = (look >> 6) - (long long)NT * ch, wi = cwd - t;
        if (cwd < 0) break;
        unsigned long long bits = 0;
        if (wi >= 0) {
            bits = ~s.claimed[wi];
            if (ch == 0 && wi == cwd) { const int top = (int)(look & 63); if (top < 63) bits &= (2ULL << top) - 1ULL; }
        }
        uint32_t total; const uint32_t off = block_excl_scan_u32<NT>((uint32_t)__popcll(bits), sm, &total);
        const uint32_t take = total >= want - got ? want - got : total;
        uint32_t k = 0;
        while (bits && off + k < take) {
            const int b = 63 - __clzll((long long)bits);
            bits &= ~(1ULL << b);
            const uint32_t id = (uint32_t)(wi * 64 + b);
            s.seedbuf[R + got + off + k] = id;
            if (off + k == take - 1) scursor = (long long)id - 1;
            k++;
        }
        got += take;
    }
    if (look < 0) got = 0;
    __threadfence();
    __syncthreads();
    if (got) cursor = scursor;
    if (t == 0) { s.rmeta[0] = R; s.rmeta[1] = assigned; s.rmeta[2] = got; }
    if (t == 0) *s.cursor = cursor < -1 ? -1 : cursor;
}
template <int NT> __global__ __launch_bounds__(NT) void k_reseed(S1Args s) { reseed_body<NT>(s); }
template <int G> __global__ __launch_bounds__(256) void k_resolve_reseed(S1Args s)
{
    resolve_body<G>(s, 0u);
    __threadfence();
    __syncthreads();
    reseed_body<256>(s);
}

#define RESEED_NT 256
#define RESEED_G 64
#ifndef RESEED_ONE_SET
#define RESEED_ONE_SET 0
#endif
#define RESEED_SPIN_LIMIT (1u << 24)
__device__ __forceinline__ void grid_meet(unsigned int *cnt, unsigned int target)
{
    __syncthreads();
    if (threadIdx.x == 0) {
        __threadfence();
        atomicAdd(cnt, 1u);
        unsigned int spins = 0;
        while (__hip_atomic_load(cnt, __ATOMIC_ACQUIRE, __HIP_MEMORY_SCOPE_AGENT) < target) {
            __builtin_amdgcn_s_sleep(2);
            if (++spins > RESEED_SPIN_LIMIT || __hip_atomic_load(cnt + 2, __ATOMIC_RELAXED, __HIP_MEMORY_SCOPE_AGENT)) { __hip_atomic_store(cnt + 2, 1u, __ATOMIC_RELAXED, __HIP_MEMORY_SCOPE_AGENT); break; }
        }
        __threadfence();
    }
    __syncthreads();
}
__global__ __launch_bounds__(RESEED_NT) void k_reseed_mg(S1Args s, unsigned int *g)
// ... 376 lines not shown
void harc_dict_free(harc_amd_ctx *c, DictDev *d)
{
    if (d->slots) harc_dev_free(c, d->slots);
    if (d->ids) harc_dev_free(c, d->ids);
    if (d->d_nbins) harc_dev_free(c, d->d_nbins);
    d->slots = nullptr; d->ids = nullptr; d->d_nbins = nullptr; d->cap = 0;
}

__global__ void k_selftest_ids(uint32_t *ids, uint32_t n)
{
    const uint32_t i = harc_gid32();
    if (i < n) ids[i] = i;
}
static int selftest_index(harc_amd_ctx *c, const uint64_t *keys, uint32_t n, uint32_t bigthresh, bool want_large, uint64_t *cap, uint32_t *nbins, void *slots,
                          uint32_t *ids, uint64_t *large, uint64_t large_capacity, uint64_t *n_large)
{
    PoolScope scope(c);
    DictDev d;
    RC_TRY(harc_dict_alloc(c, &d, n, 0));
    const uint64_t room = *cap;
    *cap = d.cap;
    if (!slots) return HARC_AMD_OK;
    if (room < d.cap) { harc_set_error("harc_amd_selftest_index: the table has %llu slots, the caller's buffer %llu", (unsigned long long)d.cap, (unsigned long long)room); return HARC_AMD_EINVAL; }
    uint64_t *k0 = nullptr; uint32_t *i0 = nullptr; unsigned long long *d_large = nullptr; unsigned int *d_nlarge = nullptr;
    const uint32_t maxlarge = 2 * (n / HARC_LARGEBIN) + 16;
    RC_TRY(dalloc(c, &k0, n)); RC_TRY(dalloc(c, &i0, n));
    if (want_large) {
        RC_TRY(dalloc(c, &d_large, maxlarge)); RC_TRY(dalloc(c, &d_nlarge, 4));
        HIP_TRY(hipMemsetAsync(d_nlarge, 0, 16, c->stream));
        d.large_list = d_large; d.large_n = d_nlarge; d.large_max = maxlarge; d.large_tag = 1u;
    }
    d.bigthresh = bigthresh;
    HIP_TRY(hipMemcpyAsync(k0, keys, (size_t)n * 8, hipMemcpyHostToDevice, c->stream));
    hipLaunchKernelGGL(k_selftest_ids, harc_grid256(n), dim3(256), 0, c->stream, i0, n);
    HIP_TRY(hipMemsetAsync(d.slots, 0xA5, d.cap * sizeof(HashSlot), c->stream));
    HIP_TRY(hipMemsetAsync(d.ids, 0xA5, (size_t)n * 4, c->stream));
    RC_TRY(harc_dict_build(c, &d, k0, i0, n, 64, HARC_KEYS_RAW));
    *nbins = d.nbins;
    HIP_TRY(hipMemcpyAsync(slots, d.slots, d.cap * sizeof(HashSlot), hipMemcpyDeviceToHost, c->stream));
    HIP_TRY(hipMemcpyAsync(ids, d.ids, (size_t)n * 4, hipMemcpyDeviceToHost, c->stream));
    unsigned int nl = 0;
    if (want_large) HIP_TRY(hipMemcpyAsync(&nl, d_nlarge, 4, hipMemcpyDeviceToHost, c->stream));
    HIP_TRY(hipStreamSynchronize(c->stream));
    if (want_large) {
        *n_large = nl;
        uint64_t take = nl < maxlarge ? nl : maxlarge;
        if (take > large_capacity) take = large_capacity;
        if (take) HIP_TRY(hipMemcpy(large, d_large, (size_t)take * 8, hipMemcpyDeviceToHost));
    }
    return HARC_AMD_OK;
}
extern "C" int harc_amd_selftest_index(harc_amd_ctx *c, const uint64_t *keys, uint64_t n, int32_t slots_per_read, uint32_t bigthresh, int32_t want_large,
                                       uint64_t *cap, uint32_t *nbins, void *slots, uint32_t *ids, uint64_t *large, uint64_t large_capacity, uint64_t *n_large)
{
    if (!c || !cap || n == 0 || n > 0xFFFFFFF0ull || (slots_per_read != 0 && (slots_per_read < 2 || slots_per_read > 4))) { harc_set_error("harc_amd_selftest_index: bad arguments"); return HARC_AMD_EINVAL; }
    if (slots && (!keys || !nbins || !ids || (want_large && (!n_large || (!large && large_capacity))))) { harc_set_error("harc_amd_selftest_index: a NULL output"); return HARC_AMD_EINVAL; }
    HIP_TRY(hipSetDevice(c->P.device));
    const int32_t spr = c->P.table_slots_per_read;
    c->P.table_slots_per_read = slots_per_read;
    const int rc = selftest_index(c, keys, (uint32_t)n, bigthresh, want_large != 0, cap, nbins, slots, ids, large, large_capacity, n_large);
    c->P.table_slots_per_read = spr;
    if (rc != HARC_AMD_OK) (void)hipStreamSynchronize(c->stream);
    return rc;
}

static std::vector<uint16_t> make_probe_table(const harc_amd_params &P)
{
    std::vector<uint16_t> t;
    for (int j = 0; j < P.maxmatch; j++) {
        for (int l = 0; l < 2; l++) if (P.dict_end[l] + j < P.readlen) t.push_back((uint16_t)(j | (0 << 8) | (l << 9)));
        for (int l = 0; l < 2; l++) if (P.dict_start[l] > j) t.push_back((uint16_t)(j | (1 << 8) | (l << 9)));
    }
    return t;
}

static uint32_t auto_chains(uint32_t N, int reads_per_chain)
{
    uint32_t k = N / (uint32_t)(reads_per_chain > 0 ? reads_per_chain : 2048);
    const uint32_t floor_k = N / 1024 < 2048 ? N / 1024 : 2048;
    if (k < floor_k) k = floor_k;
    if (k > 65536) k = 65536;
    if (k < 1) k = 1;
    return k;
}

struct EventRing {
    static constexpr int RING = 64;
    hipEvent_t ring[RING][2];
    int ring_used = 0; uint64_t ring_next = 0; double ms = 0; uint64_t launches = 0;
    EventRing() { for (int i = 0; i < RING; i++) ring[i][0] = ring[i][1] = nullptr; }
    ~EventRing() { for (int i = 0; i < ring_used; i++) { (void)hipEventDestroy(ring[i][0]); (void)hipEventDestroy(ring[i][1]); } }
    int next_pair(hipEvent_t **pair)
    {
        const int k = (int)(ring_next % RING);
        if (k >= ring_used) { HIP_TRY(hipEventCreate(&ring[k][0])); HIP_TRY(hipEventCreate(&ring[k][1])); ring_used = k + 1; }
        else RC_TRY(collect(k));
        ring_next++; launches++;
        *pair = ring[k];
        return HARC_AMD_OK;
    }
    int collect(int k) { float x = 0; HIP_TRY(hipEventSynchronize(ring[k][1])); HIP_TRY(hipEventElapsedTime(&x, ring[k][0], ring[k][1])); ms += x; return HARC_AMD_OK; }
    int collect_all() { const uint64_t n = ring_next < (uint64_t)RING ? ring_next : (uint64_t)RING; for (uint64_t i = 0; i < n; i++) RC_TRY(collect((int)i)); ring_next = 0; return HARC_AMD_OK; }
};
struct S1Resources {
    hipEvent_t e[3] = { nullptr, nullptr, nullptr };
    hipEvent_t eb[2] = { nullptr, nullptr };
    EventRing dense, coop;
    unsigned long long *h_stats = nullptr;
    ~S1Resources()
    {
        for (hipEvent_t x : e) if (x) (void)hipEventDestroy(x);
        for (hipEvent_t x : eb) if (x) (void)hipEventDestroy(x);
        if (h_stats) (void)hipHostFree(h_stats);
    }
    int init()
    {
        for (auto &x : e) HIP_TRY(hipEventCreate(&x));
        for (auto &x : eb) HIP_TRY(hipEventCreate(&x));
        HIP_TRY(hipHostMalloc((void **)&h_stats, (ST_N + HARC_COOPCNT + 8 + 1) * 8));
        return HARC_AMD_OK;
    }
};

template <int W> static int stage1_run_w(harc_amd_ctx *c)
{
    const harc_amd_params &P = c->P;
    const uint32_t N = c->N;
    uint32_t K = P.num_chains > 0 ? (uint32_t)P.num_chains : auto_chains(N, P.reads_per_chain);
    if (K > HARC_MAXK) K = HARC_MAXK;
    if (N == 0 || K > N) K = 1;
    c->C.chains = K;
    int nsteps = P.num_steps > 0 ? P.num_steps : 16;
    if (P.num_steps <= 0 && K == 1) nsteps = 64;
    if (nsteps > 64) nsteps = 64;
    bool quad = K <= 16384;
    if (const char *e = getenv("HARC_AMD_QUAD")) quad = atoi(e) != 0;
    S1Resources R;
    RC_TRY(R.init());
    hipEvent_t &e0 = R.e[0], &e1 = R.e[1], &e2 = R.e[2];
    unsigned long long *const h_stats = R.h_stats;
    HIP_TRY(hipEventRecord(e0, c->stream));

    PoolScope run_scope(c);
    RC_TRY(dalloc(c, &c->d_order, (size_t)N + 1)); RC_TRY(dalloc(c, &c->d_flag, (size_t)N + 1)); RC_TRY(dalloc(c, &c->d_pos, (size_t)N + 1));
    RC_TRY(dalloc(c, &c->d_rc, (size_t)N + 1)); RC_TRY(dalloc(c, &c->d_order_s, (size_t)N + 1));
    const harc_mark_t mark_results = harc_pool_mark(c);
    const bool itrace = getenv("HARC_AMD_TRACE") != nullptr;
    auto inow = []() { struct timespec ts; clock_gettime(CLOCK_MONOTONIC, &ts); return (double)ts.tv_sec + 1e-9 * (double)ts.tv_nsec; };
    double it0 = inow();
    auto ilap = [&](const char *what) { if (itrace) { (void)hipStreamSynchronize(c->stream); const double t = inow(); fprintf(stderr, "[index] %s: %.1f ms\n", what, 1e3 * (t - it0)); it0 = t; } };
    DictDev dict[2];
    uint32_t *d_bloom[2] = { nullptr, nullptr }; uint32_t bloom_lines = 0; int bloom_nwin[2] = { 0, 0 };
    int bloom_bits = 16, bloom_m = (P.dict_end[0] - P.dict_start[0] + 1) / 2; size_t bloom_mz_bytes = (size_t)128 << 20;
    if (bloom_m > 16) bloom_m = 16;
    if (const char *e = getenv("HARC_AMD_S1BLOOM_M")) { bloom_m = atoi(e); if (bloom_m < 0) bloom_m = 0; if (bloom_m > 16) bloom_m = 16; }
    if (const char *e = getenv("HARC_AMD_S1BLOOM_MZMB")) bloom_mz_bytes = (size_t)strtoull(e, nullptr, 10) << 20;
    const uint32_t bloom_mmask = bloom_m >= 16 ? 0xFFFFFFFFu : ((1u << (2 * bloom_m)) - 1u);
    if (const char *e = getenv("HARC_AMD_S1BLOOM")) { bloom_bits = atoi(e); if (bloom_bits < 0) bloom_bits = 0; if (bloom_bits > 64) bloom_bits = 64; }
    bool bloom_tiled = false;
    unsigned long long *d_large = nullptr; unsigned int *d_nlarge = nullptr;
    const uint32_t maxlarge = 2 * (N / HARC_LARGEBIN) + 16;
    if (N) {
        RC_TRY(harc_dict_alloc(c, &dict[0], N, 0)); RC_TRY(harc_dict_alloc(c, &dict[1], N, dict[0].cap));
        ilap("tables allocated");
        RC_TRY(dalloc(c, &d_large, maxlarge)); RC_TRY(dalloc(c, &d_nlarge, 4));
        HIP_TRY(hipMemsetAsync(d_nlarge, 0, 16, c->stream));
        for (int l = 0; l < 2; l++) { dict[l].large_list = d_large; dict[l].large_n = d_nlarge; dict[l].large_max = maxlarge; dict[l].large_tag = (uint32_t)l; }
        dict[0].bigthresh = dict[1].bigthresh = HARC_LARGEBIN;
        if (bloom_bits) {
            uint64_t nl = ((uint64_t)N * (uint64_t)bloom_bits + 511) / 512 + 1;
            if (nl > 0x0FFFFFFFull) nl = 0x0FFFFFFFull;
            bloom_lines = (uint32_t)nl;
            bloom_tiled = getenv("HARC_AMD_S1BLOOM_TILED") ? atoi(getenv("HARC_AMD_S1BLOOM_TILED")) != 0 : (size_t)bloom_lines * 64 >= ((size_t)64 << 20);
            if (((uint64_t)bloom_lines * 16 + BL_TILE_WORDS - 1) / BL_TILE_WORDS + 1 >= ((uint64_t)1 << BL_PART_BITS)) bloom_tiled = false;
            for (int l = 0; l < 2; l++) {
                RC_TRY(dalloc(c, &d_bloom[l], (size_t)bloom_lines * 16)); if (!bloom_tiled) HIP_TRY(hipMemsetAsync(d_bloom[l], 0, (size_t)bloom_lines * 64, c->stream));
                const int nb = P.dict_end[l] - P.dict_start[l] + 1;
                const bool same = P.dict_end[0] - P.dict_start[0] == P.dict_end[1] - P.dict_start[1];
                bloom_nwin[l] = (same && bloom_m > 0 && nb > bloom_m && (size_t)bloom_lines * 64 >= bloom_mz_bytes) ? nb - bloom_m + 1 : 0;
            }
        }
        PoolScope kscope(c);
        uint64_t *kboth[2] = { nullptr, nullptr }, *items[2] = { nullptr, nullptr }; uint32_t *i0 = nullptr;
        RC_TRY(dalloc(c, &kboth[0], N)); RC_TRY(dalloc(c, &kboth[1], N)); RC_TRY(dalloc(c, &i0, N));
        const bool by_items = bloom_lines && bloom_tiled;
        if (by_items) RC_TRY(dalloc(c, &items[1], N));
        const harc_mark_t mark_items1 = harc_pool_mark(c);
        if (by_items) RC_TRY(dalloc(c, &items[0], N));
        KeyOut ko[2];
        for (int l = 0; l < 2; l++)
            ko[l] = KeyOut{ kboth[l], items[l], (bloom_lines && !by_items) ? d_bloom[l] : nullptr, 2 * P.dict_start[l], 2 * (P.dict_end[l] - P.dict_start[l] + 1), bloom_nwin[l] };
        hipLaunchKernelGGL((k_keygen2<W, false>), harc_grid256(N), dim3(256), 0, c->stream, c->d_reads, N, ko[0], ko[1], i0, harc_dict_sort_bits(N), bloom_lines, bloom_mmask);
        ilap("bitmaps allocated, keys made");
        for (int l = 0; l < 2; l++) {
            const int kbits = 2 * (P.dict_end[l] - P.dict_start[l] + 1);
            if (by_items) {
                PoolScope bscope(c);
                uint64_t *pb = nullptr; RC_TRY(dalloc(c, &pb, (size_t)N + 1));
                const uint64_t nwords = (uint64_t)bloom_lines * 16;
                RC_TRY(harc_bitmap_from_items(c, items[l], pb, N, nwords, d_bloom[l]));
                if (getenv("HARC_AMD_S1BLOOM_VERIFY")) {
                    uint32_t *ref = nullptr, *ri = nullptr; unsigned long long *nd = nullptr, hnd = 0; uint64_t *raw[2] = { nullptr, nullptr };
                    RC_TRY(dalloc(c, &ref, (size_t)nwords)); RC_TRY(dalloc(c, &nd, 1)); RC_TRY(dalloc(c, &raw[0], N)); RC_TRY(dalloc(c, &raw[1], N)); RC_TRY(dalloc(c, &ri, N));
                    HIP_TRY(hipMemsetAsync(ref, 0, (size_t)nwords * 4, c->stream)); HIP_TRY(hipMemsetAsync(nd, 0, 8, c->stream));
                    KeyOut kr[2] = { ko[0], ko[1] };
                    for (int x = 0; x < 2; x++) { kr[x].keys = raw[x]; kr[x].items = nullptr; kr[x].bloom = nullptr; }
                    hipLaunchKernelGGL((k_keygen2<W, true>), harc_grid256(N), dim3(256), 0, c->stream, c->d_reads, N, kr[0], kr[1], ri, 0u, 0u, 0u);
                    hipLaunchKernelGGL(k_s1_bloom_set, harc_grid256(N), dim3(256), 0, c->stream, (const uint64_t *)raw[l], N, ref, bloom_lines, bloom_nwin[l], bloom_mmask);
                    hipLaunchKernelGGL(k_s1_bloom_diff, harc_grid256(nwords), dim3(256), 0, c->stream, (const uint32_t *)ref, (const uint32_t *)d_bloom[l], nwords, nd);
                    HIP_TRY(hipMemcpyAsync(&hnd, nd, 8, hipMemcpyDeviceToHost, c->stream));
                    HIP_TRY(hipStreamSynchronize(c->stream));
                    if (hnd) { harc_set_error("stage I bitmap built by tiles differs from the one built with atomics in %llu words", hnd); return HARC_AMD_EINTERNAL; }
                }
            }
            if (l == 0) harc_pool_release(c, mark_items1);
            ilap("bitmap built");
            RC_TRY(harc_dict_build(c, &dict[l], kboth[l], i0, N, (unsigned)kbits, HARC_KEYS_SORTABLE));
            ilap("table built");
        }
    }
    if (N && P.num_chains <= 0 && P.reads_per_chain <= 0 && (double)dict[0].nbins > 0.98 * (double)N) {
        const uint32_t k2 = N / 256 < 4096 ? N / 256 : 4096;
        if (k2 > K) { K = k2; c->C.chains = K; if (!getenv("HARC_AMD_QUAD")) quad = K <= 16384; }
    }
    uint32_t nlarge = 0;
    if (N) {
        HIP_TRY(hipMemcpyAsync(&nlarge, d_nlarge, 4, hipMemcpyDeviceToHost, c->stream));
        HIP_TRY(hipStreamSynchronize(c->stream));
        if (nlarge > maxlarge) { harc_set_error("stage I: %u bins above %u reads, list of %u", nlarge, HARC_LARGEBIN, maxlarge); return HARC_AMD_EINTERNAL; }
    }
    uint2 *d_largetab = nullptr; uint64_t *d_mirror = nullptr;
    uint32_t *d_sz0 = nullptr, *d_huge = nullptr; unsigned int *d_nhuge = nullptr; uint32_t nhuge = 0;
    uint64_t large_entries = 0;
    if (nlarge) {
        uint32_t *sz = nullptr; uint64_t *moff = nullptr;
        RC_TRY(dalloc(c, &d_largetab, nlarge)); RC_TRY(dalloc(c, &sz, (size_t)nlarge + 1)); RC_TRY(dalloc(c, &moff, (size_t)nlarge + 1));
        HIP_TRY(hipMemsetAsync(sz + nlarge, 0, 4, c->stream));
        hipLaunchKernelGGL(k_large_sizes, harc_grid256(nlarge), dim3(256), 0, c->stream, (const unsigned long long *)d_large, nlarge, dict[0].slots, dict[1].slots, sz);
        d_sz0 = sz;
        RC_TRY(dalloc(c, &d_huge, (size_t)nlarge + 1)); RC_TRY(dalloc(c, &d_nhuge, 4));
        HIP_TRY(hipMemsetAsync(d_nhuge, 0, 16, c->stream));
        hipLaunchKernelGGL(k_huge_list, harc_grid256(nlarge), dim3(256), 0, c->stream, (const uint32_t *)sz, nlarge, d_huge, d_nhuge);
        HIP_TRY(hipMemcpyAsync(&nhuge, d_nhuge, 4, hipMemcpyDeviceToHost, c->stream));
        RC_TRY(prim_excl_scan_u32_to_u64(c, sz, moff, (size_t)nlarge + 1));
        uint64_t mtotal = 0;
        HIP_TRY(hipMemcpyAsync(&mtotal, moff + nlarge, 8, hipMemcpyDeviceToHost, c->stream));
        HIP_TRY(hipStreamSynchronize(c->stream));
        if (mtotal > 0xFFFFFFFFull) { harc_set_error("stage I: more than 2^32 reads in large bins"); return HARC_AMD_EINVAL; }
        large_entries = mtotal;
        RC_TRY(dalloc(c, &d_mirror, (size_t)mtotal * W + 1));
        hipLaunchKernelGGL((k_large_fill<W>), wave_grid(nlarge), dim3(64), 0, c->stream, (const unsigned long long *)d_large, nlarge, dict[0].slots, dict[1].slots,
                           (const uint32_t *)dict[0].ids, (const uint32_t *)dict[1].ids, (const uint64_t *)moff, (const uint64_t *)c->d_reads, d_largetab, d_mirror);
        HIP_TRY(hipGetLastError());
    }
    if (P.num_steps <= 0 && K > 1) {
        const bool lowcov = N && (double)dict[0].nbins > 0.98 * (double)N;
        nsteps = ((K > 16384 || (K >= 2048 && !lowcov)) && large_entries * 50 <= (uint64_t)N) ? 32 : 16;
    }
    const bool backoff = K > 16384 && large_entries * 50 > (uint64_t)N;
    if (getenv("HARC_AMD_TRACE")) fprintf(stderr, "[stage I] %u bins of more than %u reads hold %llu entries (%.2f %% of the reads): %d steps per super-round\n", nlarge, HARC_LARGEBIN,
                                          (unsigned long long)large_entries, N ? 100.0 * (double)large_entries / (double)N : 0.0, nsteps);
    HIP_TRY(hipEventRecord(e1, c->stream));

    S1Args a; memset(&a, 0, sizeof a);
    a.L = P.readlen; a.maxmatch = P.maxmatch; a.thresh = P.thresh; a.maxsearch = P.maxsearch;
    a.Lp = ((W + 1) / 2) * 64; a.S = nsteps;
    if (backoff) { RC_TRY(dalloc(c, &a.bo, (size_t)K)); HIP_TRY(hipMemsetAsync(a.bo, 0, (size_t)K * 4, c->stream)); }
    a.nsugg_per_seed = HARC_NSUGG;
    if (K == 1) a.nsugg_per_seed = 64;
#ifdef HARC_AMD_EXPERIMENTS
    if (const char *e = getenv("HARC_AMD_NSUGG")) { a.nsugg_per_seed = atoi(e); if (a.nsugg_per_seed < 0) a.nsugg_per_seed = 0; if (a.nsugg_per_seed > HARC_NSUGG) a.nsugg_per_seed = HARC_NSUGG; }
#endif
    for (int l = 0; l < 2; l++) { a.ds[l] = P.dict_start[l]; a.de[l] = P.dict_end[l]; a.kbits[l] = 2 * (P.dict_end[l] - P.dict_start[l] + 1); }
    a.N = N; a.K = K; a.reads = c->d_reads;
    HarcComm *const cm = (c->replicated && c->comm) ? c->comm : nullptr;
    a.own_mod = cm ? (uint32_t)cm->world : 1u; a.own_rem = cm ? (uint32_t)cm->rank : 0u;
    if (a.own_mod > 64) { harc_set_error("design (R): at most 64 ranks (world %u)", a.own_mod); return HARC_AMD_EINVAL; }
    for (int l = 0; l < 2; l++) { a.slots[l] = dict[l].slots; a.cap[l] = dict[l].cap; a.ids[l] = dict[l].ids; }
    a.bloom[0] = d_bloom[0]; a.bloom[1] = d_bloom[1]; a.bloom_lines = bloom_lines; a.bloom_nwin[0] = bloom_nwin[0]; a.bloom_nwin[1] = bloom_nwin[1]; a.bloom_mmask = bloom_mmask;
    a.largetab = d_largetab; a.mirror = d_mirror;
    const size_t nwords = (size_t)N / 64 + 2;
    const uint32_t nblk = (K + 255) / 256;
    RC_TRY(dalloc(c, &a.claimed, nwords)); RC_TRY(dalloc(c, &a.bid, (size_t)N + 1)); RC_TRY(dalloc(c, &a.hdr, K));
    RC_TRY(dalloc(c, &a.cnt, (size_t)2 * K * a.Lp)); RC_TRY(dalloc(c, &a.steps, (size_t)K * 64)); RC_TRY(dalloc(c, &a.need, (size_t)K + 8192 + 1024));
    RC_TRY(dalloc(c, &a.reseed_g, 4 + 4 * RESEED_G)); HIP_TRY(hipMemsetAsync(a.reseed_g, 0, (4 + 4 * RESEED_G) * 4, c->stream));
    a.nsugg_stride = a.nsugg_per_seed > HARC_NSUGG ? a.nsugg_per_seed : HARC_NSUGG;
    RC_TRY(dalloc(c, &a.seedbuf, (size_t)K * (1 + a.nsugg_stride))); RC_TRY(dalloc(c, &a.needrank, (size_t)K + 16)); RC_TRY(dalloc(c, &a.rmeta, 4)); RC_TRY(dalloc(c, &a.cst2, (size_t)K + 1)); RC_TRY(dalloc(c, &a.sugg, (size_t)K * a.nsugg_stride));
    RC_TRY(dalloc(c, &a.slog, (size_t)N + 1));
    const size_t pg_max = (size_t)N / 64 + ((size_t)K + 1) * PG_CHUNK;
    RC_TRY(dalloc(c, &a.pg_rec, pg_max * 64)); RC_TRY(dalloc(c, &a.pg_hdr, pg_max)); RC_TRY(dalloc(c, &a.pg_cur, (size_t)K + 1)); RC_TRY(dalloc(c, &a.pg_count, 4));
    RC_TRY(dalloc(c, &a.cursor, 1)); RC_TRY(dalloc(c, &a.stats, ST_N)); RC_TRY(dalloc(c, &a.coopcnt, HARC_COOPCNT)); HIP_TRY(hipMemsetAsync(a.coopcnt, 0, HARC_COOPCNT * 8, c->stream));
    RC_TRY(dalloc(c, &a.cstat, K)); HIP_TRY(hipMemsetAsync(a.cstat, 0, (size_t)K * 16, c->stream));
    RC_TRY(dalloc(c, &a.cstat_coop, K)); HIP_TRY(hipMemsetAsync(a.cstat_coop, 0, (size_t)K * 16, c->stream)); RC_TRY(dalloc(c, &a.csteps, K)); HIP_TRY(hipMemsetAsync(a.csteps, 0, (size_t)K * 8, c->stream));
    RC_TRY(dalloc(c, &a.dbg, 48)); HIP_TRY(hipMemsetAsync(a.dbg, 0, 48 * 8, c->stream));
    unsigned long long *const dbg_ptr = a.dbg;
    if (!getenv("HARC_AMD_TRACE")) a.dbg = nullptr;
    std::vector<uint16_t> tab = make_probe_table(P);
    uint16_t *d_tab = nullptr; RC_TRY(dalloc(c, &d_tab, tab.size() + 1));
    HIP_TRY(hipMemcpyAsync(d_tab, tab.data(), tab.size() * 2, hipMemcpyHostToDevice, c->stream));
    a.probe_tab = d_tab; a.nprobe = (int)tab.size();
    {
        uint32_t *lt = nullptr;
        const size_t nm = (size_t)2 * P.maxmatch * StepsLds<W>::MROW;
        RC_TRY(dalloc(c, &lt, nm + 2 * tab.size() + 2));
        hipLaunchKernelGGL((k_steps_tables<W>), dim3(4), dim3(256), 0, c->stream, a, lt);
        a.lds_tab = lt;
    }
    a.stepcap = HARC_STEP_CAP; a.budget = HARC_SCAN_BUDGET;
#ifdef HARC_AMD_EXPERIMENTS
    if (getenv("HARC_AMD_STEPCAP")) a.stepcap = atoi(getenv("HARC_AMD_STEPCAP"));
    if (getenv("HARC_AMD_BUDGET")) a.budget = atoi(getenv("HARC_AMD_BUDGET"));
#endif
    if (a.stepcap < 1) a.stepcap = 1;
    a.weedmin = getenv("HARC_AMD_WEEDMIN") ? atoi(getenv("HARC_AMD_WEEDMIN")) : 3;
    a.lazy = getenv("HARC_AMD_LAZY") ? (atoi(getenv("HARC_AMD_LAZY")) != 0 ? 1 : 0) : 1;
    a.firstmax = (bloom_nwin[0] > 0 && bloom_nwin[1] > 0) ? 64 : 48;
    if (const char *e = getenv("HARC_AMD_FIRSTMAX")) { const int x = atoi(e); a.firstmax = x < 1 ? 1 : x > 64 ? 64 : x; }
    {
        bool want = getenv("HARC_AMD_SUCC") ? atoi(getenv("HARC_AMD_SUCC")) != 0 : K == 1;
        const size_t sbytes = (size_t)N * 2 * HARC_SUCC_N * sizeof(uint2);
        size_t fr = 0, tot = 0;
        if (want) HIP_TRY(hipMemGetInfo(&fr, &tot));
        if (want && N && quad && !cm && a.lazy && P.maxsearch >= (int)HARC_LARGEBIN && P.thresh <= 127 && a.nprobe <= 4095 && P.maxmatch <= 255 && sbytes < tot / 8) {
            uint2 *sp = nullptr;
            RC_TRY(dalloc(c, &sp, (size_t)N * 2 * HARC_SUCC_N));
            hipLaunchKernelGGL((k_succ<W>), harc_fold256(((uint64_t)N * 2 + 3) / 4), dim3(256), succ_lds_bytes(W, P.maxmatch, a.nprobe), c->stream, a, sp, N);
            HIP_TRY(hipGetLastError());
            a.succ = sp;
            if (getenv("HARC_AMD_TRACE")) fprintf(stderr, "[stage I] successor lists of %u reads x 2 orientations (%.1f MB)\n", N, (double)sbytes / 1e6);
        }
    }
    HIP_TRY(hipMemsetAsync(a.claimed, 0, nwords * 8, c->stream));
    HIP_TRY(hipMemsetAsync(a.bid, 0xFF, ((size_t)N + 1) * 4, c->stream));
    HIP_TRY(hipMemsetAsync(a.slog, 0xFF, ((size_t)N + 1) * sizeof(uint2), c->stream));
    HIP_TRY(hipMemsetAsync(a.rmeta, 0, 16, c->stream));
    HIP_TRY(hipMemsetAsync(a.stats, 0, ST_N * 8, c->stream));
    HIP_TRY(hipMemsetAsync(a.need, 0, (size_t)K + 8192 + 1024, c->stream));
    const long long cur0 = (long long)N - 1;
    HIP_TRY(hipMemcpyAsync(a.cursor, &cur0, 8, hipMemcpyHostToDevice, c->stream));
    {
        const unsigned long long act0 = N == 0 ? 0ULL : (N / K > 0 ? (unsigned long long)K : 1ULL);
        HIP_TRY(hipMemcpyAsync(a.stats + ST_ACTIVE, &act0, 8, hipMemcpyHostToDevice, c->stream));
    }
    hipLaunchKernelGGL(k_init_chains, dim3(nblk), dim3(256), 0, c->stream, a);
    HIP_TRY(hipGetLastError());

    if (nlarge) hipLaunchKernelGGL((k_compact_bins<W>), wave_grid(nlarge), dim3(64), 0, c->stream, a, (const unsigned long long *)d_large, nlarge, (const uint32_t *)d_sz0);
    if (nhuge) hipLaunchKernelGGL((k_compact_huge<W>), dim3(nhuge), dim3(1024), 0, c->stream, a, (const unsigned long long *)d_large, (const uint32_t *)d_huge, nhuge);
    uint32_t *x_send = nullptr, *x_recv = nullptr; uint32_t x_nper = 0; size_t x_bytes = 0; unsigned long long *x_dig = nullptr;
    std::vector<size_t> x_so, x_sb, x_ro, x_rb;
    if (cm) {
        x_nper = ((((K + 3) / 4) + a.own_mod - 1) / a.own_mod) * 4;
        x_bytes = (size_t)x_nper * (8 + 2 * (size_t)nsteps) * 4;
        RC_TRY(dalloc(c, &x_send, x_bytes / 4 + 4)); RC_TRY(dalloc(c, &x_recv, (x_bytes / 4) * a.own_mod + 4));
        x_so.assign(a.own_mod, 0); x_sb.assign(a.own_mod, x_bytes); x_ro.resize(a.own_mod); x_rb.assign(a.own_mod, x_bytes);
        for (uint32_t p = 0; p < a.own_mod; p++) x_ro[p] = (size_t)p * x_bytes;
        RC_TRY(dalloc(c, &x_dig, 8));
    }
    const size_t lds_bytes = steps_lds_bytes(W, P.maxmatch, a.nprobe), lds_bytes_seq = steps_lds_bytes(W, P.maxmatch, a.nprobe, true), lds_bytes_coop = steps_lds_bytes_coop(W, P.maxmatch, a.nprobe);
    const bool prof = P.profile != 0;
    bool seq = getenv("HARC_AMD_SEQ") ? atoi(getenv("HARC_AMD_SEQ")) != 0 : (HARC_SEQ_SCAN && N && (double)dict[0].nbins > 0.88 * (double)N);
    const bool spec = (getenv("HARC_AMD_SPEC") ? atoi(getenv("HARC_AMD_SPEC")) != 0 : true) && W >= 4 && a.kbits[0] == 64 && a.kbits[1] == 64 && bloom_lines > 0 && bloom_nwin[0] == 17 && bloom_nwin[1] == 17 &&
                      bloom_mmask == 0xFFFFFFFFu && (dict[0].cap >> 34) == 0 && P.maxsearch >= (int)HARC_LARGEBIN && a.firstmax == 64;
    int seq_probe = (!getenv("HARC_AMD_SEQ") && HARC_SEQ_SCAN && !quad && seq) ? 0 : 2;
    float seq_ms[2] = { 0, 0 };
    const uint64_t seq_key = ((uint64_t)N << 32) ^ ((uint64_t)K << 8) ^ ((uint64_t)nsteps << 1) ^ ((uint64_t)P.readlen << 52) ^ 1u;
    bool seq_measured = false;
    if (seq_probe == 0 && c->s1_seq_key == seq_key && c->s1_seq_choice >= 0 && !(getenv("HARC_AMD_SEQ_REMEASURE") && atoi(getenv("HARC_AMD_SEQ_REMEASURE")) != 0)) { seq = c->s1_seq_choice != 0; seq_probe = 2; }
    uint64_t rounds = 0, launches = 0;
    int coop_forced = getenv("HARC_AMD_COOP_WAVES") ? atoi(getenv("HARC_AMD_COOP_WAVES")) : 0;
    if (coop_forced != 1 && coop_forced != 2 && coop_forced != 4) coop_forced = 0;
    int coop_waves = coop_forced ? coop_forced : 4;
    unsigned long long coop_seen = 0;
    double coop_slots = 1024.0;
    { hipDeviceProp_t pr; if (hipGetDeviceProperties(&pr, P.device) == hipSuccess && pr.multiProcessorCount > 0) coop_slots = 4.0 * pr.multiProcessorCount; }
    const int batch = getenv("HARC_AMD_BATCHSYNC") ? atoi(getenv("HARC_AMD_BATCHSYNC")) : (K <= 4 ? 32 : 8);
    const bool reseed_mg = getenv("HARC_AMD_RESEED_MG") ? atoi(getenv("HARC_AMD_RESEED_MG")) != 0 : K > 4096;
    const bool fused_rr = !reseed_mg && K <= 4u * (64u / (nsteps <= 16 ? 16u : nsteps <= 32 ? 32u : 64u)) && !(getenv("HARC_AMD_FUSED_RR") && atoi(getenv("HARC_AMD_FUSED_RR")) == 0);
    a.reseed_win = RESEED_G * RESEED_NT;
    if (const char *e = getenv("HARC_AMD_RESEED_WIN")) { const int x = atoi(e); if (x >= 1 && x <= RESEED_G * RESEED_NT) a.reseed_win = (uint32_t)x; }
    if (const char *e = getenv("HARC_AMD_RESEED_STRESS")) { const int x = atoi(e); a.reseed_stress = x < 0 ? 0u : x > 1000 ? 1000u : (uint32_t)x; }
    for (;;) {
        if (seq_probe < 2) { seq = seq_probe == 0; HIP_TRY(hipEventRecord(R.eb[0], c->stream)); }
        for (int r = 0; r < batch; r++) {
            hipEvent_t *pair = nullptr;
            if (cm) hipLaunchKernelGGL(k_apply_seed, dim3(nblk), dim3(256), 0, c->stream, a);
            if (prof) { RC_TRY(R.dense.next_pair(&pair)); HIP_TRY(hipEventRecord(pair[0], c->stream)); }
            if (quad) hipLaunchKernelGGL((k_steps<W, true, false>), dim3((K + 3) / 4), dim3(256), lds_bytes_seq, c->stream, a);
            else if (seq && spec) hipLaunchKernelGGL((k_steps<W, false, false, 4, true, true>), dim3((K + 3) / 4), dim3(256), lds_bytes_seq, c->stream, a);
            else if (seq) hipLaunchKernelGGL((k_steps<W, false, false, 4, true>), dim3((K + 3) / 4), dim3(256), lds_bytes_seq, c->stream, a);
            else hipLaunchKernelGGL((k_steps<W, false, false>), dim3((K + 3) / 4), dim3(256), lds_bytes, c->stream, a);
            if (prof) HIP_TRY(hipEventRecord(pair[1], c->stream));
            if (nlarge) {
                if (prof) { RC_TRY(R.coop.next_pair(&pair)); HIP_TRY(hipEventRecord(pair[0], c->stream)); }
                if (coop_waves == 1) hipLaunchKernelGGL((k_steps<W, true, true, 1>), dim3(K), dim3(64), lds_bytes_coop, c->stream, a);
                else if (coop_waves == 2) hipLaunchKernelGGL((k_steps<W, true, true, 2>), dim3(K), dim3(128), lds_bytes_coop, c->stream, a);
                else hipLaunchKernelGGL((k_steps<W, true, true>), dim3(K), dim3(256), lds_bytes_coop, c->stream, a);
                if (prof) HIP_TRY(hipEventRecord(pair[1], c->stream));
            }
            if (cm) {
                const uint64_t tot = (uint64_t)x_nper * (8 + 2 * (uint64_t)nsteps);
                hipLaunchKernelGGL(k_pack_chains, harc_grid256(tot), dim3(256), 0, c->stream, a, x_send, x_nper);
                const void *sp[1] = { x_send }; void *rp[1] = { x_recv };
                const size_t *sop[1] = { x_so.data() }, *sbp[1] = { x_sb.data() }, *rop[1] = { x_ro.data() }, *rbp[1] = { x_rb.data() };
                RC_TRY(cm->alltoallv(c, 1, sp, sop, sbp, rp, rop, rbp));
                hipLaunchKernelGGL(k_unpack_chains, dim3((unsigned)((tot + 255) / 256), a.own_mod), dim3(256), 0, c->stream, a, (const uint32_t *)x_recv, x_nper);
            }
            if (fused_rr) {
                if (nsteps <= 16) hipLaunchKernelGGL((k_resolve_reseed<16>), dim3(1), dim3(256), 0, c->stream, a);
                else if (nsteps <= 32) hipLaunchKernelGGL((k_resolve_reseed<32>), dim3(1), dim3(256), 0, c->stream, a);
                else hipLaunchKernelGGL((k_resolve_reseed<64>), dim3(1), dim3(256), 0, c->stream, a);
            }
            else if (nsteps <= 16) hipLaunchKernelGGL((k_resolve<16>), dim3((K + 15) / 16), dim3(256), 0, c->stream, a);
            else if (nsteps <= 32) hipLaunchKernelGGL((k_resolve<32>), dim3((K + 7) / 8), dim3(256), 0, c->stream, a);
            else hipLaunchKernelGGL((k_resolve<64>), dim3((K + 3) / 4), dim3(256), 0, c->stream, a);
            if (fused_rr) { }
            else if (reseed_mg) hipLaunchKernelGGL(k_reseed_mg, dim3(RESEED_G), dim3(RESEED_NT), 0, c->stream, a, a.reseed_g);
            else if (K <= 4096) hipLaunchKernelGGL((k_reseed<256>), dim3(1), dim3(256), 0, c->stream, a);
            else hipLaunchKernelGGL((k_reseed<1024>), dim3(1), dim3(1024), 0, c->stream, a);
            if (nlarge) hipLaunchKernelGGL((k_compact_bins<W>), wave_grid(nlarge), dim3(64), 0, c->stream, a, (const unsigned long long *)d_large, nlarge, (const uint32_t *)d_sz0);
    if (nhuge) hipLaunchKernelGGL((k_compact_huge<W>), dim3(nhuge), dim3(1024), 0, c->stream, a, (const unsigned long long *)d_large, (const uint32_t *)d_huge, nhuge);
            launches++;
        }
        rounds += batch;
        if (seq_probe < 2) HIP_TRY(hipEventRecord(R.eb[1], c->stream));
        HIP_TRY(hipMemcpyAsync(h_stats, a.stats, ST_N * 8, hipMemcpyDeviceToHost, c->stream));
        if (nlarge) HIP_TRY(hipMemcpyAsync(h_stats + ST_N, a.coopcnt, HARC_COOPCNT * 8, hipMemcpyDeviceToHost, c->stream));
        unsigned int *const h_reseed_timeout = reinterpret_cast<unsigned int *>(h_stats + ST_N + HARC_COOPCNT + 8);
        *h_reseed_timeout = 0;
        if (reseed_mg) HIP_TRY(hipMemcpyAsync(h_reseed_timeout, a.reseed_g + 2, 4, hipMemcpyDeviceToHost, c->stream));
        if (cm) {
            HIP_TRY(hipMemsetAsync(x_dig, 0, 8 * 8, c->stream));
            hipLaunchKernelGGL(k_replica_digest, dim3(1024), dim3(256), 0, c->stream, a, (unsigned long long)nwords, x_dig);
            HIP_TRY(hipMemcpyAsync(h_stats + ST_N + HARC_COOPCNT, x_dig, 8 * 8, hipMemcpyDeviceToHost, c->stream));
            RC_TRY(cm->wait(c, "all-gather of the walked steps"));
        }
        HIP_TRY(hipStreamSynchronize(c->stream));
        HIP_TRY(hipGetLastError());
        if (*h_reseed_timeout) { harc_set_error("stage I: the workgroups of k_reseed_mg did not meet (super-round %llu); HARC_AMD_RESEED_MG=0 uses the single workgroup", (unsigned long long)rounds); return HARC_AMD_EINTERNAL; }
        if (seq_probe < 2) {
            HIP_TRY(hipEventElapsedTime(&seq_ms[seq_probe], R.eb[0], R.eb[1]));
            if (++seq_probe == 2) { seq = seq_ms[0] < seq_ms[1]; seq_measured = true; }
        }
        if (nlarge && coop_forced == 0) {
            unsigned long long tot = 0;
            for (int k = 0; k < HARC_COOPCNT; k++) tot += h_stats[ST_N + k];
            const double per_round = (double)(tot - coop_seen) / (double)batch;
            coop_seen = tot;
            coop_waves = per_round > 5.0 * coop_slots ? 1 : per_round > 3.0 * coop_slots ? 2 : 4;
        }
        if (cm) {
            uint64_t mine[10], all[10 * 64];
            for (int k = 0; k < 7; k++) mine[k] = h_stats[ST_N + HARC_COOPCNT + k];
            mine[7] = h_stats[ST_ACTIVE];
            mine[8] = seq_probe == 2 ? (seq ? 1u : 0u) : 2u; mine[9] = (uint64_t)coop_waves;
            RC_TRY(cm->allgather_u64(c, mine, 10, all));
            static const char *const what[8] = { "claim bitmap", "chain headers", "chains asking for a seed", "cursor", "seeds wanted", "seeds handed out", "look-ahead seeds", "chains alive" };
            for (uint32_t p = 0; p < a.own_mod; p++) for (int k = 0; k < 8; k++) if (all[(size_t)p * 10 + k] != all[k]) {
                harc_set_error("design (R): the replicas of rank 0 and rank %u differ after super-round %llu (%s: %llx / %llx)", p, (unsigned long long)rounds, what[k],
                               (unsigned long long)all[k], (unsigned long long)all[(size_t)p * 10 + k]);
                return HARC_AMD_EINTERNAL;
            }
            if (all[8] < 2u) seq = all[8] != 0;
            if (coop_forced == 0 && (all[9] == 1u || all[9] == 2u || all[9] == 4u)) coop_waves = (int)all[9];
        }
        if (seq_measured) { c->s1_seq_key = seq_key; c->s1_seq_choice = seq ? 1 : 0; seq_measured = false; }
        if (getenv("HARC_AMD_TRACE")) {
            uint32_t rm[4] = { 0, 0, 0, 0 };
            HIP_TRY(hipMemcpy(rm, a.rmeta, 16, hipMemcpyDeviceToHost));
            fprintf(stderr, "[stage I] round %llu: %llu chains alive%s; extra passes of k_reseed_mg so far %u\n", (unsigned long long)rounds, h_stats[ST_ACTIVE], seq ? " (wave-uniform scan)" : "", rm[3]);
        }
        if (h_stats[ST_ACTIVE] == 0) break;
        if (rounds > (uint64_t)N * 2 + 1024) { harc_set_error("stage I did not converge after %llu rounds", (unsigned long long)rounds); return HARC_AMD_EINTERNAL; }
    }
    HIP_TRY(hipEventRecord(e2, c->stream));

    uint32_t *nmain = nullptr, *nsing = nullptr, *bmain = nullptr, *bsing = nullptr;
    RC_TRY(dalloc(c, &nmain, (size_t)K + 1)); RC_TRY(dalloc(c, &nsing, (size_t)K + 1)); RC_TRY(dalloc(c, &bmain, (size_t)K + 1)); RC_TRY(dalloc(c, &bsing, (size_t)K + 1));
    HIP_TRY(hipMemsetAsync(nmain, 0, ((size_t)K + 1) * 4, c->stream)); HIP_TRY(hipMemsetAsync(nsing, 0, ((size_t)K + 1) * 4, c->stream));
    hipLaunchKernelGGL(k_chain_counts, dim3(nblk), dim3(256), 0, c->stream, a.hdr, a.cstat, (const uint4 *)a.cstat_coop, (const uint2 *)a.csteps, (const uint2 *)a.cst2, K, nmain, nsing, a.stats);
    RC_TRY(prim_excl_scan_u32(c, nmain, bmain, (size_t)K + 1));
    RC_TRY(prim_excl_scan_u32(c, nsing, bsing, (size_t)K + 1));
    uint32_t M = 0, S = 0; const unsigned long long nlog = N;
    HIP_TRY(hipMemcpyAsync(&M, bmain + K, 4, hipMemcpyDeviceToHost, c->stream));
    HIP_TRY(hipMemcpyAsync(&S, bsing + K, 4, hipMemcpyDeviceToHost, c->stream));
    unsigned int npages = 0;
    HIP_TRY(hipMemcpyAsync(&npages, a.pg_count, 4, hipMemcpyDeviceToHost, c->stream));
    HIP_TRY(hipStreamSynchronize(c->stream));
    if (getenv("HARC_AMD_DIAG")) {
        std::vector<unsigned long long> hc(nwords); std::vector<uint32_t> hb((size_t)N + 1); std::vector<ChainHdr> hh(K);
        HIP_TRY(hipMemcpy(hc.data(), a.claimed, nwords * 8, hipMemcpyDeviceToHost));
        HIP_TRY(hipMemcpy(hb.data(), a.bid, ((size_t)N + 1) * 4, hipMemcpyDeviceToHost)); HIP_TRY(hipMemcpy(hh.data(), a.hdr, (size_t)K * sizeof(ChainHdr), hipMemcpyDeviceToHost));
        unsigned long long nunclaimed = 0, nact = 0, npend = 0;
        for (uint32_t k = 0; k < K; k++) { if (hh[k].flags & CH_ACTIVE) nact++; if (hh[k].flags & CH_PREVUNM) npend++; }
        for (unsigned long long i = 0; i < nlog; i++) {
            if ((hc[i >> 6] >> (i & 63)) & 1ULL) continue;
            if (nunclaimed++ < 24) fprintf(stderr, "[diag rank %u] read %llu was never claimed; bid %x\n", a.own_rem, i, hb[i]);
        }
        fprintf(stderr, "[diag rank %u] %llu reads unclaimed; M %u S %u N %u; chains active %llu, with a pending seed %llu; rounds %llu\n", a.own_rem, nunclaimed, M, S, N, nact, npend, (unsigned long long)rounds);
    }
    if ((unsigned long long)M + S != nlog) { harc_set_error("stage I bookkeeping: M=%u S=%u N=%u", M, S, N); return HARC_AMD_EINTERNAL; }
    c->M = M; c->S = S;
    unsigned long long *d_found = a.stats + ST_N - 1;
    if (nlog) hipLaunchKernelGGL(k_s1_singles, dim3((unsigned)(nlog / 256 + 1 < 8192 ? nlog / 256 + 1 : 8192)), dim3(256), 0, c->stream, (const uint2 *)a.slog, nlog, K, bsing, c->d_order_s, d_found);
    if ((size_t)npages > pg_max) { harc_set_error("stage I bookkeeping: %u pages handed out, %zu reserved", npages, pg_max); return HARC_AMD_EINTERNAL; }
    if (npages) hipLaunchKernelGGL(k_pages_out, dim3((npages + 3) / 4), dim3(256), 0, c->stream, (const uint2 *)a.pg_rec, (const uint2 *)a.pg_hdr, (uint32_t)npages, (const uint32_t *)nmain, (const uint32_t *)bmain,
                                   c->d_order, c->d_flag, c->d_pos, c->d_rc);
    HIP_TRY(hipGetLastError());
    HIP_TRY(hipMemcpyAsync(h_stats, a.stats, ST_N * 8, hipMemcpyDeviceToHost, c->stream));
    HIP_TRY(hipStreamSynchronize(c->stream));
    if (h_stats[ST_N - 1] != S) { harc_set_error("stage I bookkeeping: %llu singleton records for %u singletons", h_stats[ST_N - 1], S); return HARC_AMD_EINTERNAL; }

    c->C.n_main = M; c->C.n_singleton = S; c->C.unmatched = h_stats[ST_UNMATCHED]; c->C.conflicts = h_stats[ST_CONFLICTS];
    c->C.probes = h_stats[ST_PROBES]; c->C.candidates = h_stats[ST_CANDS]; c->C.useful_probes = h_stats[ST_USEFUL]; c->C.candidates_seq = h_stats[ST_CANDS_SEQ]; c->C.rounds = rounds; c->C.propose_launches = launches;
    float ms = 0;
    HIP_TRY(hipEventElapsedTime(&ms, e0, e1)); c->C.index_ms = ms;
    HIP_TRY(hipEventElapsedTime(&ms, e1, e2)); c->C.chain_ms = ms;
    RC_TRY(R.dense.collect_all()); RC_TRY(R.coop.collect_all());
    c->C.propose_ms = R.dense.ms;
    c->C.coop_ms = R.coop.ms; c->C.coop_launches = R.coop.launches;
    c->C.coop_useful_probes = h_stats[ST_COOP_USEFUL]; c->C.coop_candidates_seq = h_stats[ST_COOP_CANDS_SEQ]; c->C.coop_candidates = h_stats[ST_COOP_CANDS];
    c->C.coop_steps = h_stats[ST_COOP_STEPS]; c->C.dense_steps = h_stats[ST_DENSE_STEPS];
#ifdef HARC_TIMING
    {
        unsigned long long d[16];
        HIP_TRY(hipMemcpy(d, a.dbg, sizeof d, hipMemcpyDeviceToHost));
        const double st = (double)(d[6] ? d[6] : 1);
        fprintf(stderr, "[k_steps timing] steps %llu waves-launched %llu; cycles/step: top %.0f pack+rc %.0f probe+smallscan %.0f coop %.0f bid %.0f update %.0f\n",
                d[6], d[7], d[0] / st, d[1] / st, d[2] / st, d[3] / st, d[4] / st, d[5] / st);
        fprintf(stderr, "[k_steps timing] per step: batches %.2f  max-lane slot iterations %.2f  max-lane scan iterations %.2f  total scan iterations %.2f  lanes probing %.1f\n",
                d[10] / st, d[8] / st, d[9] / st, d[11] / st, d[12] / st);
    }
#endif
    if (a.dbg) {
        unsigned long long d[48];
        HIP_TRY(hipMemcpy(d, dbg_ptr, sizeof d, hipMemcpyDeviceToHost));
#ifdef HARC_SKETCH_STATS
        fprintf(stderr, "[sketch] Hamming tests of the cooperative scans: %llu; passed %llu (%.3f %%); a 16-base sketch would have rejected %llu (%.1f %%), a 32-base sketch %llu (%.1f %%)\n", d[44], d[47], 100.0 * (double)d[47] / (double)(d[44] ? d[44] : 1),
                d[45], 100.0 * (double)d[45] / (double)(d[44] ? d[44] : 1), d[46], 100.0 * (double)d[46] / (double)(d[44] ? d[44] : 1));
#endif
        const double stp = (double)(d[4] ? d[4] : 1);
        fprintf(stderr, "[k_steps] steps walked %llu (of them kept %u): per step batches %.2f, cooperative bin scans %.2f, their 64-entry chunks %.2f, chunk x probe tests %.2f; steps without a hit %.3f\n", d[4], N, d[5] / stp, d[0] / stp, d[1] / stp, d[3] / stp, d[2] / stp);
        fprintf(stderr, "[k_steps] worst walk of the run: %llu chunks, %llu chunk x probe tests, %llu bin scans\n", d[6], d[7], d[8]);
        fprintf(stderr, "[k_steps] walks of the main kernel: %llu (%.0f per super-round); %llu of them end in front of a large bin (%.1f %%), %llu of those without a step walked (%.1f %% of all walks)\n",
                d[13], (double)d[13] / (double)(rounds ? rounds : 1), d[15], 100.0 * (double)d[15] / (double)(d[13] ? d[13] : 1), d[14], 100.0 * (double)d[14] / (double)(d[13] ? d[13] : 1));
        if (d[9]) fprintf(stderr, "[k_steps] cooperative walks: %llu (%.1f per super-round), %.2f steps each, mean %.1f us, longest %.1f us (100 MHz wall clock)\n",
                          d[9], (double)d[9] / (double)(rounds ? rounds : 1), (double)d[12] / (double)d[9], (double)d[10] / (double)d[9] / 100.0, (double)d[11] / 100.0);
        if (d[9] && d[16]) {
            fprintf(stderr, "[k_steps] cooperative walks, mean us by phase: setup %.1f, consensus rows %.1f, probes + small bins %.1f, large-bin scans %.1f, bid + update %.1f, tail %.1f\n",
                    d[16] / (double)d[9] / 100.0, d[17] / (double)d[9] / 100.0, d[18] / (double)d[9] / 100.0, d[19] / (double)d[9] / 100.0, d[20] / (double)d[9] / 100.0, d[21] / (double)d[9] / 100.0);
            fprintf(stderr, "[k_steps] large-bin scans by live entries of the bin: <= 64: %llu (%.2f us each), <= 256: %llu (%.2f), <= 1024: %llu (%.2f), more: %llu (%.2f)\n",
                    d[36], d[40] / (double)(d[36] ? d[36] : 1) / 100.0, d[37], d[41] / (double)(d[37] ? d[37] : 1) / 100.0, d[38], d[42] / (double)(d[38] ? d[38] : 1) / 100.0, d[39], d[43] / (double)(d[39] ? d[39] : 1) / 100.0);
            fprintf(stderr, "[k_steps] cooperative walks by duration (25 us bins, last = longer):");
            for (int k = 0; k < 12; k++) fprintf(stderr, " %llu", d[24 + k]);
            fprintf(stderr, "\n");
        }
    }

    harc_pool_release(c, mark_results);
    run_scope.keep();
    c->have_s1 = true;
    return HARC_AMD_OK;
}

template <int W> static int orient_w(harc_amd_ctx *c, const uint64_t *reads, const uint32_t *order, const uint8_t *rc, uint32_t m, uint64_t *out)
{
    if (!m) return HARC_AMD_OK;
    { const uint32_t per_block = 4u * (64u / W); hipLaunchKernelGGL((k_orient<W>), harc_fold256(((uint64_t)m + per_block - 1) / per_block), dim3(256), 0, c->stream, reads, order, rc, m, c->P.readlen, out); }
    HIP_TRY(hipGetLastError());
    return HARC_AMD_OK;
}
int s1_orient(harc_amd_ctx *c, const uint64_t *reads, const uint32_t *order, const uint8_t *rc, uint32_t m, uint64_t *out)
{
    switch (c->W) {
    case 1: return orient_w<1>(c, reads, order, rc, m, out);
    case 2: return orient_w<2>(c, reads, order, rc, m, out);
    case 3: return orient_w<3>(c, reads, order, rc, m, out);
    case 4: return orient_w<4>(c, reads, order, rc, m, out);
    case 5: return orient_w<5>(c, reads, order, rc, m, out);
    case 6: return orient_w<6>(c, reads, order, rc, m, out);
    case 7: return orient_w<7>(c, reads, order, rc, m, out);
    default: return orient_w<8>(c, reads, order, rc, m, out);
    }
}

int stage1_run(harc_amd_ctx *c)
{
    switch (c->W) {
    case 1: return stage1_run_w<1>(c);
    case 2: return stage1_run_w<2>(c);
    case 3: return stage1_run_w<3>(c);
    case 4: return stage1_run_w<4>(c);
    case 5: return stage1_run_w<5>(c);
    case 6: return stage1_run_w<6>(c);
    case 7: return stage1_run_w<7>(c);
    default: return stage1_run_w<8>(c);
    }
}

int stage1_make_oriented(harc_amd_ctx *c, uint32_t i0, uint32_t i1)
{
    if (!c->d_oreads) RC_TRY(dalloc(c, &c->d_oreads, (size_t)c->M * c->W + 1));
    if (i1 > c->M) i1 = c->M;
    if (i0 >= i1) return HARC_AMD_OK;
    return s1_orient(c, c->d_reads, c->d_order + i0, c->d_rc + i0, i1 - i0, c->d_oreads + (size_t)i0 * c->W);
}
```

Measured before the change: 710.3.

## Carry probe-batch hash lookups across exact-match steps in spec seq kernel

New measurement: 746.1, median of 6. +5.0%, better.

```diff
diff --git a/harc_amd/csrc/stage1.hip b/harc_amd/csrc/stage1.hip
--- a/harc_amd/csrc/stage1.hip
+++ b/harc_amd/csrc/stage1.hip
@@ -644,10 +644,11 @@
     const int NW = 2 * W, ROW = 3 * NW + 1, MROW = (NW + 3) & ~3;
     return ((size_t)2 * maxmatch * MROW + (size_t)((2 * ROW + 3) & ~3) + (size_t)MROW + (size_t)8 * NW + (size_t)32 + (size_t)2 * nprobe + 8) * 4 + HARC_WGCMD_BYTES + 16;
 }
-static inline size_t steps_lds_bytes(int W, int maxmatch, int nprobe, bool seq = false)
+#define HARC_CARRY_DW (4 * (64 * 2 + 2))
+static inline size_t steps_lds_bytes(int W, int maxmatch, int nprobe, bool seq = false, bool carry = false)
 {
     const int NW = 2 * W, ROW = 3 * NW + 1, MROW = (NW + 3) & ~3;
-    return (size_t)4 * (64 * ((W + 1) / 2)) * 16 + ((size_t)2 * maxmatch * MROW + (size_t)4 * 2 * ROW + (size_t)4 * MROW + (size_t)4 * 8 * NW + (size_t)4 * 32 + (size_t)(seq ? 4 * HARC_OWN_SLOTS : 0) + (size_t)2 * nprobe + 8) * 4 + 32;
+    return (carry ? (size_t)(HARC_CARRY_DW + 2 * maxmatch) * 4 : 0) + (size_t)4 * (64 * ((W + 1) / 2)) * 16 + ((size_t)2 * maxmatch * MROW + (size_t)4 * 2 * ROW + (size_t)4 * MROW + (size_t)4 * 8 * NW + (size_t)4 * 32 + (size_t)(seq ? 4 * HARC_OWN_SLOTS : 0) + (size_t)2 * nprobe + 8) * 4 + 32;
 }
 template <int W> __device__ __forceinline__ int ham_window(const uint32_t *row, int bitoff, const uint32_t *mrow, const uint32_t (&rd)[2 * W])
 {
@@ -1085,6 +1086,18 @@
         const int hoff = dir * ROW * 32 + 32 * NW + (dir ? -2 * j : 2 * j);
         pinfo[i] = make_uint2((uint32_t)koff | ((uint32_t)dir << 13) | ((uint32_t)l << 14) | ((uint32_t)j << 16),
                               (uint32_t)hoff | ((uint32_t)((dir * s.maxmatch + j) * MROW) << 16));
+    }
+    uint32_t *const cmap = out + nm + 2 * s.nprobe;
+    for (int i = blockIdx.x * blockDim.x + threadIdx.x; i < 2 * s.maxmatch; i += gridDim.x * blockDim.x) {
+        uint32_t w = 0;
+        for (int b = 0; b < 2; b++) {
+            const int e = 2 * i + b, g = e / s.maxmatch, j = e % s.maxmatch;
+            const uint32_t want = (uint32_t)j | ((uint32_t)(g & 1) << 8) | ((uint32_t)(g >> 1) << 9);
+            uint32_t q = 0xFFFFu;
+            for (int p = 0; p < s.nprobe && p < 0xFFFF; p++) if (s.probe_tab[p] == want) q = (uint32_t)p;
+            w |= q << (16 * b);
+        }
+        cmap[i] = w;
     }
 }
 
@@ -1201,6 +1214,8 @@
     constexpr int NW = StepsLds<W>::NW, ROW = StepsLds<W>::ROW, MROW = StepsLds<W>::MROW;
     extern __shared__ __attribute__((aligned(16))) uint32_t lds[];
     constexpr int NSL = COOP ? 1 : 4;
+    constexpr bool CARRY = SEQ && SPEC && !COOP && !QUAD && W >= 4 && HARC_SEQ_OWNT;
+    constexpr int OWNSTRIDE = HARC_OWN_SLOTS + (CARRY ? HARC_CARRY_DW / 4 : 0);
     uint32_t *const s_mask = lds + (COOP ? (size_t)0 : (size_t)4 * ConsState<W, !QUAD>::LP * 4);
     uint32_t *const s_rows = s_mask + (size_t)2 * s.maxmatch * MROW;
     uint32_t *const s_rdl = s_rows + ((NSL * 2 * ROW + 3) & ~3);
@@ -1208,7 +1223,7 @@
     uint32_t *const s_pend = s_tmp + NSL * 8 * NW;
     uint32_t *const s_own = s_pend + NSL * 32;
     constexpr bool OWNT = (SEQ && HARC_SEQ_OWNT) || (QUAD && !COOP);
-    uint2 *const s_pinfo = reinterpret_cast<uint2 *>(s_own + (OWNT ? 4 * HARC_OWN_SLOTS : 0));
+    uint2 *const s_pinfo = reinterpret_cast<uint2 *>(s_own + (OWNT ? 4 * OWNSTRIDE : 0));
     WgCmd *const cmd = reinterpret_cast<WgCmd *>(reinterpret_cast<char *>(s_pinfo + s.nprobe) + 8 - ((size_t)(s_pinfo + s.nprobe) & 7));
     const int lane = threadIdx.x & 63, role = threadIdx.x >> 6, wv = COOP ? 0 : role;
     const int L = s.L;
@@ -1223,9 +1238,12 @@
         for (int i = threadIdx.x; i < nm; i += 64 * NWV) s_mask[i] = s.lds_tab[i];
         const uint2 *const pt = reinterpret_cast<const uint2 *>(s.lds_tab + nm);
         for (int i = threadIdx.x; i < s.nprobe; i += 64 * NWV) s_pinfo[i] = pt[i];
+        if constexpr (CARRY) {
+            for (int i = threadIdx.x; i < 2 * s.maxmatch; i += 64 * NWV) reinterpret_cast<uint32_t *>(s_pinfo + s.nprobe)[i] = s.lds_tab[nm + 2 * s.nprobe + i];
+        }
         for (int i = threadIdx.x; i < NSL * 2 * ROW; i += 64 * NWV) s_rows[i] = 0u;
         for (int i = threadIdx.x; i < NSL * 8 * NW; i += 64 * NWV) s_tmp[i] = 0u;
-        if constexpr (OWNT) for (int i = threadIdx.x; i < 4 * HARC_OWN_SLOTS; i += 64 * NWV) s_own[i] = HARC_NONE;
+        if constexpr (OWNT) for (int i = threadIdx.x; i < 4 * OWNSTRIDE; i += 64 * NWV) s_own[i] = HARC_NONE;
         __syncthreads();
     }
     if (COOP && role != 0) {
@@ -1264,9 +1282,13 @@
         h.n_main = (uint32_t)__builtin_amdgcn_readfirstlane((int)h1.x); h.n_sing = (uint32_t)__builtin_amdgcn_readfirstlane((int)h1.y);
         h.nsteps = (uint32_t)__builtin_amdgcn_readfirstlane((int)h1.z); h.pad0 = (uint32_t)__builtin_amdgcn_readfirstlane((int)h1.w);
     }
-    uint4 cst = s.cstat[c];
-    cst.x = (uint32_t)__builtin_amdgcn_readfirstlane((int)cst.x); cst.y = (uint32_t)__builtin_amdgcn_readfirstlane((int)cst.y);
-    cst.z = (uint32_t)__builtin_amdgcn_readfirstlane((int)cst.z); cst.w = (uint32_t)__builtin_amdgcn_readfirstlane((int)cst.w);
+    constexpr bool CST_LATE = CARRY;
+    uint4 cst = make_uint4(0, 0, 0, 0);
+    if constexpr (!CST_LATE) {
+        cst = s.cstat[c];
+        cst.x = (uint32_t)__builtin_amdgcn_readfirstlane((int)cst.x); cst.y = (uint32_t)__builtin_amdgcn_readfirstlane((int)cst.y);
+        cst.z = (uint32_t)__builtin_amdgcn_readfirstlane((int)cst.z); cst.w = (uint32_t)__builtin_amdgcn_readfirstlane((int)cst.w);
+    }
     if (!(h.flags & CH_ACTIVE)) return;
     if (!COOP && s.bo && (s.bo[c] & 0xFFu)) return;
     if (COOP && !(h.flags & CH_COOP)) return;
@@ -1277,7 +1299,8 @@
             h.n_sing++;
         }
         if (r < assigned) {
-            const uint32_t id = s.seedbuf[r];
+            uint32_t id = s.seedbuf[r];
+            if constexpr (CARRY) id = (uint32_t)__builtin_amdgcn_readfirstlane((int)id);
             h.cur = id; h.prev = id; h.flags = ((h.flags | CH_PREVUNM) & ~CH_NEEDSEED) & 0xFFFFu; h.mode = 2;
             const uint32_t first = r * (uint32_t)s.nsugg_per_seed;
             const uint32_t ng = first >= got ? 0u : (got - first < (uint32_t)s.nsugg_per_seed ? got - first : (uint32_t)s.nsugg_per_seed);
@@ -1333,11 +1356,14 @@
 
     uint32_t *const rowF = s_rows + (size_t)wv * 2 * ROW, *const rowR = rowF + ROW, *const rdl = s_rdl + (size_t)wv * MROW;
     uint8_t *const coltmp = reinterpret_cast<uint8_t *>(s_tmp + (size_t)wv * 8 * NW);
-    uint32_t *const ownt = s_own + (size_t)wv * HARC_OWN_SLOTS;
+    uint32_t *const ownt = s_own + (size_t)wv * OWNSTRIDE;
+    uint2 *const stash = reinterpret_cast<uint2 *>(ownt + HARC_OWN_SLOTS); uint32_t *const cmeta = ownt + HARC_OWN_SLOTS + 128;
     uint16_t *const pshift = reinterpret_cast<uint16_t *>(s_pend + (size_t)wv * 32);
     const uint64_t kmask0 = (SPEC || s.kbits[0] >= 64) ? ~(uint64_t)0 : (((uint64_t)1 << s.kbits[0]) - 1), kmask1 = (SPEC || s.kbits[1] >= 64) ? ~(uint64_t)0 : (((uint64_t)1 << s.kbits[1]) - 1);
     const uint64_t cap = s.cap[0];
     uint32_t dbg_bins = 0, dbg_iter = 0, dbg_miss = 0, dbg_surv = 0, dbg_batches = 0;
+    uint32_t wk = 0;
+#define VACC(x, inc) do { asm volatile("" : "+v"(x)); (x) += (inc); } while (0)
     uint32_t np = 0, nc = 0, nuse = 0, ncu = 0;
     using flag_t = typename std::conditional<SEQ, int, bool>::type;
     int nst = 0; flag_t needseed = false, defer = false;
@@ -1347,7 +1373,7 @@
     const int resume = (int)(h.flags >> 16);
     flag_t stalled = false; int resume_next = 0;
     flag_t rows_ok = false; int pend = 0, ptot = 0;
-    const flag_t lazy = (SEQ || (QUAD && !COOP)) && s.lazy != 0;
+    const flag_t lazy = CARRY ? (flag_t)s.lazy : (flag_t)((SEQ || (QUAD && !COOP)) && s.lazy != 0);
     constexpr bool FASTP = QUAD && !COOP;
     uint32_t lastrid = HARC_NONE; int lastdir = 0; bool rows_lazy = false;
     uint2 enext = make_uint2(HARC_NONE, 0u); bool have_next = false;
@@ -1424,12 +1450,15 @@
         PH(1);
         int base = (t == 0 && resume > 0) ? resume : 0;
         int stepbig = 0;
-        for (int bi = 0; base < s.nprobe; bi++) {
+        int bi0 = 0;
+        if constexpr (CARRY) { if (__builtin_amdgcn_readfirstlane((int)*cmeta) >= 0) bi0 = -1; }
+        int bi = bi0;
+        for (; base < s.nprobe; bi++) {
             int bend;
-            { int w0 = bi == 0 ? ((HARC_W0_MUL * (lastp >> 4) + HARC_W0_ADD + 15) & ~15) : 64; const int wmax = (QUAD || SPEC) ? 64 : (bi <= 1 ? s.firstmax : 64); if (w0 > wmax) w0 = wmax; bend = base + w0; }
+            { int w0 = bi <= 0 ? ((HARC_W0_MUL * (lastp >> 4) + HARC_W0_ADD + 15) & ~15) : 64; const int wmax = (QUAD || SPEC) ? 64 : (bi <= 1 ? s.firstmax : 64); if (w0 > wmax) w0 = wmax; bend = base + w0; }
             if (bend > s.nprobe) bend = s.nprobe;
             if (bend <= base) bend = s.nprobe;
-            const int p = base + lane; dbg_batches++;
+            const int p = base + lane; if constexpr (!CARRY) dbg_batches++;
             uint32_t mine = HARC_NONE; int j = 0, dir = 0, l = 0, myhd = 0;
             uint32_t pix = 0;
             uint32_t ncb = 0;
@@ -1437,6 +1466,27 @@
             uint2 b_lt = make_uint2(0, 0);
             bool cand = false; uint32_t c_sst = 0, c_cw = 0, c_piy = 0; uint64_t c_slot = 0;
             uint32_t mrd[NW];
+            if (CARRY && bi < 0) {
+                const uint32_t cm = (uint32_t)__builtin_amdgcn_readfirstlane((int)*cmeta);
+                bool known = false;
+                int ln = lane; asm volatile("" : "+v"(ln));
+                if (ln < s.nprobe) {
+                    const uint2 pi = s_pinfo[ln];
+                    const uint32_t jn = (pi.x >> 16) + (cm & 0xFFu);
+                    if (jn < (uint32_t)s.maxmatch) {
+                        const uint32_t qb = reinterpret_cast<const uint16_t *>(s_pinfo + s.nprobe)[((pi.x >> 13) & 3u) * (uint32_t)s.maxmatch + jn], q = qb - (cm >> 8);
+                        if (qb != 0xFFFFu && q < 64u) {
+                            const uint2 e = stash[q];
+                            if (e.y != HARC_NONE) { known = true; pix = pi.x; c_piy = pi.y; c_sst = e.x; c_cw = e.y; cand = e.y != 0u; }
+                        }
+                    }
+                }
+                const unsigned long long unk = ~__ballot(known);
+                bend = unk ? __ffsll((long long)unk) - 1 : 64;
+                if (lane >= bend) cand = false;
+                if (cand && (c_cw & SLOT_EMB) && own_has(ownt, c_sst)) { cand = false; c_cw = 0u; }
+                if (lane == 0) *cmeta = HARC_NONE;
+            } else
             if (p < bend && (SPEC || cap)) {
                 const uint2 pi = s_pinfo[p];
                 pix = pi.x;
@@ -1514,6 +1564,7 @@
                         if (cw & SLOT_EMB) {
                             if (__popcll(__ballot(true)) >= s.weedmin && ((reinterpret_cast<const uint32_t *>(s.claimed)[sst >> 5] >> (sst & 31u)) & 1u)) { cand = false; atomicOr(reinterpret_cast<uint32_t *>(&tab[sl + qhit]) + 3, SLOT_DEAD); }
                             else if (OWNT && own_has(ownt, sst)) cand = false;
+                            if constexpr (CARRY) c_cw = cand ? c_cw : 0u;
                         }
                     }
                     else {
@@ -1548,10 +1599,17 @@
                 }
             }
             int winlane = 64;
+            if constexpr (CARRY) { if (p >= bend) c_cw = HARC_NONE; }
             if constexpr (SEQ) {
             {
                 unsigned long long mc = __ballot(cand);
-                if (!COOP) { const unsigned long long mb = __ballot(big); if (mb) mc &= (mb & (0ULL - mb)) - 1ULL; }
+                if (!COOP) {
+                    const unsigned long long mb = __ballot(big);
+                    if (mb) {
+                        mc &= (mb & (0ULL - mb)) - 1ULL;
+                        if constexpr (CARRY) { if (lane >= __ffsll((long long)mb) - 1) c_cw = HARC_NONE; }
+                    }
+                }
                 const bool exactwin = !SPEC && s.maxsearch < (int)HARC_LARGEBIN;
                 uint32_t ntest = 0;
                 while (mc) {
@@ -1570,6 +1628,7 @@
                     uint32_t lead = 0, hit = HARC_NONE, rd = 0; bool alltop = true; int seen = 0, hit_hd = -1;
                     uint32_t idv = 0;
                     if (!emb && (uint32_t)lane < cntb) idv = ids[o_sst + lane];
+                    if constexpr (CARRY) asm volatile("" : "+v"(idv));
                     for (uint32_t i = cntb; i > 0 && seen < s.maxsearch; i--) {
                         const uint32_t rid = emb ? o_sst : (uint32_t)__builtin_amdgcn_readlane((int)idv, (int)(i - 1));
                         if (!OWNT && __ballot(ownreg == rid && lane < t)) { alltop = false; continue; }
@@ -1589,7 +1648,7 @@
                         ntest++; if (exactwin) seen++;
                         if (hd <= s.thresh) { hit = rid; hit_hd = hd; break; }
                     }
-                    if (lead && lane == 0) {
+                    if (lead && lane == 0 && !(CARRY && bi < 0)) {
                         uint32_t *cp = reinterpret_cast<uint32_t *>(&(o_l ? s.slots[1] : s.slots[0])[o_slot]) + 3;
                         if (lead == cntb) atomicOr(cp, SLOT_DEAD); else if (!emb) atomicMin(cp, (cntb - lead) | (o_cw & SLOT_OVF));
                     }
@@ -1618,7 +1677,7 @@
                 const unsigned long long bigall = __ballot(big);
                 unsigned long long bigm = bigall;
                 if (winlane < 64) bigm &= (1ULL << winlane) - 1ULL;
-                if (!COOP) { if (bigm) { defer = true; break; } }
+                if (!COOP) { if (bigm) { defer = true; if constexpr (CARRY) bi++; break; } }
                 int caplane = 64;
                 if (COOP) {
                     const int need = s.stepcap - stepbig;
@@ -1668,16 +1727,25 @@
             PH(3);
             if (lane <= winlane) ncu += ncb;
             if (found != HARC_NONE) {
-                nuse += (uint32_t)(base + winlane + 1);
+                if constexpr (CARRY) VACC(nuse, (uint32_t)(base + winlane + 1)); else nuse += (uint32_t)(base + winlane + 1);
                 lastp += 4 * (base + winlane) - (lastp >> 2);
+                if constexpr (CARRY) {
+                    if ((lazy & 2) && fhd == 0) {
+                        int ln = lane; asm volatile("" : "+v"(ln));
+                        stash[ln] = make_uint2(c_sst, c_cw);
+                        if (lane == 0) *cmeta = ((uint32_t)base << 8) | (uint32_t)fj;
+                    }
+                    bi++;
+                }
                 break;
             }
             base = bend;
         }
+        if constexpr (CARRY) VACC(wk, (uint32_t)bi << 16);
         }
         if (defer || stalled) break;
         if (found == HARC_NONE) {
-            nuse += (uint32_t)s.nprobe; dbg_miss++;
+            if constexpr (CARRY) { VACC(nuse, (uint32_t)s.nprobe); VACC(wk, 1u << 8); } else { nuse += (uint32_t)s.nprobe; dbg_miss++; }
             if (ownlate && own_ins < t) own_sync(t);
             uint32_t sid = HARC_NONE;
             if (spos < nsugg) {
@@ -1690,7 +1758,7 @@
                     else for (int k = 0; k < t; k++) okc = okc && ((uint32_t)__builtin_amdgcn_readlane((int)ownreg, k) != id);
                 }
                 const unsigned long long sm = __ballot(okc);
-                if (sm) { const int f = __ffsll((long long)sm) - 1; sid = __shfl(id, f, 64); spos += f + 1; } else spos = nsugg;
+                if (sm) { const int f = __ffsll((long long)sm) - 1; if constexpr (CARRY) sid = (uint32_t)__builtin_amdgcn_readlane((int)id, f); else sid = __shfl(id, f, 64); spos += f + 1; } else spos = nsugg;
             }
             if (sid == HARC_NONE) { needseed = true; break; }
             if (lane == 0) s.steps[(size_t)c * 64 + t] = make_uint2(sid, (1u << 16) | ((uint32_t)spos << 24));
@@ -1701,10 +1769,11 @@
                 if (lane < NW) { const uint32_t *rp = reinterpret_cast<const uint32_t *>(s.reads + (size_t)sid * W); rdl[lane] = rp[lane]; }
                 __builtin_amdgcn_fence(__ATOMIC_RELEASE, "wavefront");
                 __builtin_amdgcn_wave_barrier();
-                cons_reset_lds(st, rdl, L, lane);
+                int ln = lane; if constexpr (CARRY) asm volatile("" : "+v"(ln));
+                cons_reset_lds(st, rdl, L, ln);
             }
             rows_ok = false; pend = 0; ptot = 0;
-            nst++;
+            if constexpr (CARRY) VACC(wk, 1u); else nst++;
             if (COOP && bigprobes >= s.budget) break;
             continue;
         }
@@ -1738,10 +1807,12 @@
                 if (FASTP) { lastrid = HARC_NONE; rows_lazy = false; }
             }
         }
-        nst++;
+        if constexpr (CARRY) VACC(wk, 1u); else nst++;
         PH(4);
         if (COOP && bigprobes >= s.budget) break;
     }
+    if constexpr (CARRY) { wk = (uint32_t)__builtin_amdgcn_readfirstlane((int)wk); nst = (int)(wk & 0xFFu); dbg_miss = (wk >> 8) & 0xFFu; dbg_batches = wk >> 16; nuse = (uint32_t)__builtin_amdgcn_readfirstlane((int)nuse); }
+#undef VACC
     if (lane >= T0 && lane < T0 + nst) atomicMin(&s.bid[ownreg], ((uint32_t)lane << 20) | c);
     if (ownlate) counts_sync();
     if (pend) {
@@ -1767,7 +1838,7 @@
     if (lane == 0 && s.dbg) { atomicAdd(&s.dbg[0], (unsigned long long)dbg_bins); atomicAdd(&s.dbg[1], (unsigned long long)dbg_iter); atomicAdd(&s.dbg[2], (unsigned long long)dbg_miss); atomicAdd(&s.dbg[3], (unsigned long long)dbg_surv); atomicAdd(&s.dbg[4], (unsigned long long)nst); atomicAdd(&s.dbg[5], (unsigned long long)dbg_batches); atomicMax(&s.dbg[6], (unsigned long long)dbg_iter); atomicMax(&s.dbg[7], (unsigned long long)dbg_surv); atomicMax(&s.dbg[8], (unsigned long long)dbg_bins); }
     if (lane == 0) {
         if (COOP) { atomicAdd(&s.cstat_coop[c].x, np); atomicAdd(&s.cstat_coop[c].y, nc); atomicAdd(&s.cstat_coop[c].z, nuse); atomicAdd(&s.cstat_coop[c].w, ncu); s.csteps[c].y += (uint32_t)nst; }
-        else { cst.x += np; cst.y += nc; cst.z += nuse; cst.w += ncu; s.cstat[c] = cst; s.csteps[c].x += (uint32_t)nst; }
+        else { if constexpr (CST_LATE) cst = s.cstat[c]; cst.x += np; cst.y += nc; cst.z += nuse; cst.w += ncu; s.cstat[c] = cst; s.csteps[c].x += (uint32_t)nst; }
         h.mode = 0;
         h.nsteps = (h.nsteps & 0xFFFF0000u) | (uint32_t)(T0 + nst);
         h.pad0 = ((uint32_t)lastp & 0xFFFFu) | (((uint32_t)spos & 0xFFu) << 16) | (widebits << 24);
@@ -2750,7 +2821,7 @@
     {
         uint32_t *lt = nullptr;
         const size_t nm = (size_t)2 * P.maxmatch * StepsLds<W>::MROW;
-        RC_TRY(dalloc(c, &lt, nm + 2 * tab.size() + 2));
+        RC_TRY(dalloc(c, &lt, nm + 2 * tab.size() + 2 + 2 * (size_t)P.maxmatch));
         hipLaunchKernelGGL((k_steps_tables<W>), dim3(4), dim3(256), 0, c->stream, a, lt);
         a.lds_tab = lt;
     }
@@ -2762,6 +2833,7 @@
     if (a.stepcap < 1) a.stepcap = 1;
     a.weedmin = getenv("HARC_AMD_WEEDMIN") ? atoi(getenv("HARC_AMD_WEEDMIN")) : 3;
     a.lazy = getenv("HARC_AMD_LAZY") ? (atoi(getenv("HARC_AMD_LAZY")) != 0 ? 1 : 0) : 1;
+    if (a.lazy && !(getenv("HARC_AMD_CARRY") && atoi(getenv("HARC_AMD_CARRY")) == 0) && a.nprobe < 0xFFFF && P.maxmatch <= 255) a.lazy |= 2;
     a.firstmax = (bloom_nwin[0] > 0 && bloom_nwin[1] > 0) ? 64 : 48;
     if (const char *e = getenv("HARC_AMD_FIRSTMAX")) { const int x = atoi(e); a.firstmax = x < 1 ? 1 : x > 64 ? 64 : x; }
     {
@@ -2805,7 +2877,7 @@
         for (uint32_t p = 0; p < a.own_mod; p++) x_ro[p] = (size_t)p * x_bytes;
         RC_TRY(dalloc(c, &x_dig, 8));
     }
-    const size_t lds_bytes = steps_lds_bytes(W, P.maxmatch, a.nprobe), lds_bytes_seq = steps_lds_bytes(W, P.maxmatch, a.nprobe, true), lds_bytes_coop = steps_lds_bytes_coop(W, P.maxmatch, a.nprobe);
+    const size_t lds_bytes = steps_lds_bytes(W, P.maxmatch, a.nprobe), lds_bytes_seq = steps_lds_bytes(W, P.maxmatch, a.nprobe, true), lds_bytes_carry = steps_lds_bytes(W, P.maxmatch, a.nprobe, true, true), lds_bytes_coop = steps_lds_bytes_coop(W, P.maxmatch, a.nprobe);
     const bool prof = P.profile != 0;
     bool seq = getenv("HARC_AMD_SEQ") ? atoi(getenv("HARC_AMD_SEQ")) != 0 : (HARC_SEQ_SCAN && N && (double)dict[0].nbins > 0.88 * (double)N);
     const bool spec = (getenv("HARC_AMD_SPEC") ? atoi(getenv("HARC_AMD_SPEC")) != 0 : true) && W >= 4 && a.kbits[0] == 64 && a.kbits[1] == 64 && bloom_lines > 0 && bloom_nwin[0] == 17 && bloom_nwin[1] == 17 &&
@@ -2835,7 +2907,7 @@
             if (cm) hipLaunchKernelGGL(k_apply_seed, dim3(nblk), dim3(256), 0, c->stream, a);
             if (prof) { RC_TRY(R.dense.next_pair(&pair)); HIP_TRY(hipEventRecord(pair[0], c->stream)); }
             if (quad) hipLaunchKernelGGL((k_steps<W, true, false>), dim3((K + 3) / 4), dim3(256), lds_bytes_seq, c->stream, a);
-            else if (seq && spec) hipLaunchKernelGGL((k_steps<W, false, false, 4, true, true>), dim3((K + 3) / 4), dim3(256), lds_bytes_seq, c->stream, a);
+            else if (seq && spec) hipLaunchKernelGGL((k_steps<W, false, false, 4, true, true>), dim3((K + 3) / 4), dim3(256), lds_bytes_carry, c->stream, a);
             else if (seq) hipLaunchKernelGGL((k_steps<W, false, false, 4, true>), dim3((K + 3) / 4), dim3(256), lds_bytes_seq, c->stream, a);
             else hipLaunchKernelGGL((k_steps<W, false, false>), dim3((K + 3) / 4), dim3(256), lds_bytes, c->stream, a);
             if (prof) HIP_TRY(hipEventRecord(pair[1], c->stream));
```
